# pierremtb/PINNs-TF2.0

Hardware: AMD Instinct MI355X
Metric: collocation-points/sec (higher is better)
Workload: dtype f64

## Files before the change

include/pinn_hip.h:

```cpp
#ifndef PINN_HIP_H
#define PINN_HIP_H

#include <stdint.h>

#ifdef __cplusplus
extern "C" {
#endif

typedef struct pinn_ctx pinn_ctx;

enum {
  PINN_PDE_BURGERS = 0,
  PINN_PDE_BURGERS_IDE = 1,
  PINN_PDE_SCHRODINGER = 2,
  PINN_PDE_BURGERS_DISC = 3,
  PINN_PDE_BURGERS_DISC_IDE = 4,
  PINN_PDE_ADR = 5,
  PINN_PDE_ADR_IDE = 6
};
enum { PINN_F32 = 0, PINN_F64 = 1 };
enum {
  PINN_OK = 0, PINN_EINVAL = -1, PINN_EHIP = -2, PINN_ESTATE = -3, PINN_ECOMM = -4,
  PINN_EUNSUPPORTED = -5
};

const char* pinn_last_error(void);
int pinn_abi_version(void);
int pinn_device_count(int* n);
int pinn_runtime_versions(int* hip_runtime, int* hip_driver, int* rccl);
int pinn_device_info(int device, char* name, int cap, int* n_cu, int64_t* hbm_bytes);

int pinn_create(pinn_ctx** out, const int* layers, int n_layers, const double* lb,
                const double* ub, int pde_kind, int dtype, int device);
int pinn_destroy(pinn_ctx* c);
int pinn_num_params(pinn_ctx* c, int64_t* n);

int pinn_set_collocation(pinn_ctx* c, const double* X_f, int64_t n, int64_t n_total);
int pinn_set_data(pinn_ctx* c, const double* X_u, const double* u, int64_t n, int64_t n_total);
int pinn_lhs_collocation(pinn_ctx* c, int64_t n_design, int64_t first, int64_t count, uint64_t seed);
int pinn_get_collocation(pinn_ctx* c, double* X, int64_t n);
int pinn_rad_collocation(pinn_ctx* c, int64_t n_design, int64_t first, int64_t count, int64_t n_pool, uint64_t seed,
                         int k, double c_add);
int pinn_set_boundary(pinn_ctx* c, const double* X_lb, const double* X_ub, int64_t n,
                      int64_t n_total);
int pinn_disc_set_stage(pinn_ctx* c, int set, const double* x, const double* target, int64_t n,
                        const double* M, int q);
int pinn_disc_predict(pinn_ctx* c, int set, const double* x, int64_t n, double* out);

int pinn_set_pde_params(pinn_ctx* c, const double* p, int n);
int pinn_get_pde_params(pinn_ctx* c, double* p, int n);
int pinn_set_pde_trainable(pinn_ctx* c, int mask);

int pinn_set_weights(pinn_ctx* c, const double* w, int64_t n);
int pinn_get_weights(pinn_ctx* c, double* w, int64_t n);

int pinn_loss_grad(pinn_ctx* c, double* loss, double* grad, double* terms);

int pinn_adam_init(pinn_ctx* c, double lr, double beta1, double beta2, double eps);
int pinn_adam_run(pinn_ctx* c, int n_steps, double* losses);
int pinn_adam_run_terms(pinn_ctx* c, int n_steps, double* terms3);

int pinn_lbfgs_begin(pinn_ctx* c, int max_iter, double lr, int n_corr, double tol_fun,
                     double tol_x, double max_eval);
int pinn_lbfgs_run(pinn_ctx* c, int n_iters, int* iters, double* losses, int* n_logged,
                   int* done);
int pinn_adam_enqueue(pinn_ctx* c, int n_steps, int* ticket);
int pinn_adam_enqueue_terms(pinn_ctx* c, int n_steps, int* ticket);
int pinn_adam_collect(pinn_ctx* c, int ticket, double* losses);
int pinn_lbfgs_enqueue(pinn_ctx* c, int n_iters, int* ticket);
int pinn_lbfgs_collect(pinn_ctx* c, int ticket, int cap, int* iters, double* losses, int* n_logged, int* done);
int pinn_weights_snapshot(pinn_ctx* c, int slot);
int pinn_weights_restore(pinn_ctx* c, int slot);
int pinn_lbfgs_set_mode(pinn_ctx* c, int mode);
int pinn_lbfgs_get_x(pinn_ctx* c, double* x, int64_t n);

int pinn_predict(pinn_ctx* c, const double* X, int64_t n, double* out);
int pinn_error_l2(pinn_ctx* c, const double* X, const double* ref, int64_t n, int kind, double* err);
int pinn_residual(pinn_ctx* c, double* f, int64_t n);
int pinn_residual_at(pinn_ctx* c, const double* X, int64_t n, double* f);

int pinn_get_status(pinn_ctx* c, int64_t* n_evals, int64_t* first_nonfinite_eval);

int pinn_comm_unique_id(char* id128);
int pinn_comm_init(pinn_ctx* c, const char* id128, int n_ranks, int rank);
int pinn_comm_xgmi_export(pinn_ctx* c, int n_ranks, int rank, char* handle64);
int pinn_comm_xgmi_attach(pinn_ctx* c, const char* handles, int n_handles, int* mapped_ok);
int pinn_comm_xgmi_selftest(pinn_ctx* c, int* ok);
int pinn_comm_benchmark(pinn_ctx* c, int mode, int iters, double* us_per_iter);
int pinn_comm_set_mode(pinn_ctx* c, int mode);
int pinn_comm_get_mode(pinn_ctx* c, int* mode);

int pinn_timing_enable(pinn_ctx* c, int max_evals, int every);
int pinn_timing_read(pinn_ctx* c, double* avg_ms, int* n);
int pinn_sync(pinn_ctx* c);
int pinn_set_kernel_path(pinn_ctx* c, int path);
int pinn_get_kernel_path(pinn_ctx* c, int* path);
int pinn_debug_stamps(pinn_ctx* c, long long* out, int64_t cap, int64_t* n_waves);
int pinn_debug_coef_stamps(long long* out16);
int pinn_debug_t16f_stamps(long long* out512);
int pinn_debug_t16_deal(int W, int* out49);

typedef struct pinn_ens pinn_ens;
int pinn_ens_create(pinn_ens** out, const int* layers, int n_layers, const double* lb, const double* ub, int pde_kind,
                    int dtype, int device, int n_members);
int pinn_ens_destroy(pinn_ens* e);
int pinn_ens_size(pinn_ens* e, int* n_members, int64_t* n_params);
int pinn_ens_set_collocation(pinn_ens* e, const double* X_f, int64_t n, int64_t n_total);
int pinn_ens_set_data(pinn_ens* e, const double* X_u, const double* u, int64_t n, int64_t n_total);
int pinn_ens_set_pde_params(pinn_ens* e, const double* p, int n);
int pinn_ens_set_weights(pinn_ens* e, const double* w, int64_t n);
int pinn_ens_get_weights(pinn_ens* e, double* w, int64_t n);
int pinn_ens_loss_grad(pinn_ens* e, double* losses, double* grads, double* terms);
int pinn_ens_adam_init(pinn_ens* e, double lr, double beta1, double beta2, double eps, const double* lr_k);
int pinn_ens_adam_run(pinn_ens* e, int n_steps, double* losses);
int pinn_ens_lbfgs_begin(pinn_ens* e, int n_corr, double tol_fun, double tol_x, double max_eval, double lr,
                         const double* lr_k, int max_iter, const int* max_iter_k);
int pinn_ens_lbfgs_run(pinn_ens* e, int n_iters, int* iters, double* losses, int* n_logged, int* done);
int pinn_ens_predict(pinn_ens* e, const double* X, int64_t n, double* out);
int pinn_ens_error_l2(pinn_ens* e, const double* X, const double* ref, int64_t n, double* err);
int pinn_ens_get_status(pinn_ens* e, int64_t* n_evals, int64_t* first_nonfinite_eval);

int pinn_ensk_set_collocation(pinn_ens* e, const double* X_f, int64_t n, int64_t n_total);
int pinn_ensk_set_data(pinn_ens* e, const double* X_u, const double* u, int64_t n, int64_t n_total);
int pinn_ensk_set_pde_params(pinn_ens* e, const double* nu, int n_members);
int pinn_ensk_lhs_collocation(pinn_ens* e, int64_t n_design, int64_t first, int64_t count, const uint64_t* seeds);

int pinn_sa_set_weights(pinn_ctx* c, const double* lam_u, int64_t n_u, const double* lam_f, int64_t n_f);
int pinn_sa_get_weights(pinn_ctx* c, double* lam_u, int64_t n_u, double* lam_f, int64_t n_f);
int pinn_sa_adam_init(pinn_ctx* c, double lr);
int pinn_sa_disable(pinn_ctx* c);

int pinn_pw_set(pinn_ctx* c, const double* lam_u, int64_t n_u, const double* lam_f, int64_t n_f, const double* lam_b,
                int64_t n_b);
int pinn_pw_get(pinn_ctx* c, double* lam_u, int64_t n_u, double* lam_f, int64_t n_f, double* lam_b, int64_t n_b);
int pinn_pw_adam_init(pinn_ctx* c, double rate_u, double rate_f, double rate_b);
int pinn_pw_disable(pinn_ctx* c);

int pinn_set_robin(pinn_ctx* c, const double* X_w , const double* alpha, const double* beta, const double* g,
                   int64_t n, int64_t n_total);
int pinn_robin_residual(pinn_ctx* c, double* out , int64_t n);

int pinn_set_source(pinn_ctx* c, const double* s , int64_t n);

int pinn_set_coef_fields(pinn_ctx* c, const double* K , int64_t n);

#ifdef __cplusplus
}
#endif
#endif
```

pinns-tf2.0_amd/csrc/engine.hip:

```cpp
#include <hip/hip_runtime.h>
#include <rccl/rccl.h>

#include <cmath>
#include <cstdarg>
#include <cstddef>
#include <cstdio>
#include <cstring>
#include <string>
#include <chrono>
#include <vector>

#include "../../include/pinn_hip.h"
#include "kernels_fused20.h"
#include "kernels_fused20m.h"
#include "fused20d_api.h"
#include "fused20m_api.h"
#include "kernels_wide.h"
#include "kernels_generic.h"
#include "kernels_optim.h"
#include "kernels_disc.h"
#include "kernels_sampling.h"
#include "kernels_rad.h"
#include "kernels_tile16.h"
#include "kernels_tile16f.h"
// ... 26 lines not shown

#define NCCLCHK(expr)                                                                     \
  do {                                                                                    \
    ncclResult_t r_ = (expr);                                                             \
    if (r_ != ncclSuccess)                                                                \
      return fail(PINN_ECOMM, "%s failed: %s (%s:%d)", #expr, ncclGetErrorString(r_),     \
                  __FILE__, __LINE__);                                                    \
  } while (0)

#define REQUIRE(cond, ...)                                \
  do {                                                    \
    if (!(cond)) return fail(PINN_EINVAL, __VA_ARGS__);   \
  } while (0)

struct Roctx {
  int (*push)(const char*) = nullptr;
  int (*pop)() = nullptr;
  Roctx() {
    if (getenv("PINN_NO_ROCTX")) return;
    void* h = dlopen("librocprofiler-sdk-roctx.so", RTLD_LAZY | RTLD_GLOBAL);
    if (!h) h = dlopen("librocprofiler-sdk-roctx.so.1", RTLD_LAZY | RTLD_GLOBAL);
    if (!h) return;
    push = (int (*)(const char*))dlsym(h, "roctxRangePushA");
    pop = (int (*)())dlsym(h, "roctxRangePop");
    if (!push || !pop) push = nullptr, pop = nullptr;
  }
};
static Roctx& roctx() { static Roctx r; return r; }
struct Range {
  bool on;
  explicit Range(const char* name) : on(roctx().push != nullptr) { if (on) roctx().push(name); }
  ~Range() { if (on) roctx().pop(); }
};

static constexpr int CHUNK_POINTS = 32768;
static constexpr int LOSS_SLOTS = 4;

enum KernelPath : int {
  KP_GENERIC = 0,
  KP_FUSED20 = 1,
  KP_FUSED20M = 2,
  KP_WIDE = 3,
  KP_T16 = 4,
  KP_T16_FWD = 5,
  KP_T16_BWD = 6,
  KP_FUSED20D = 7,
  KP_T16_FUSED = 8,
  KP_COUNT
};

enum { LAM_PAIRS, LAM_DATA, LAM_COL, LAM_CLASSES };
struct LamStore {
  double* buf = nullptr;
  size_t cap = 0;
  int n_hdr = 0;
  double hdr[PW_CONST] = {0.0, 0.0, 0.0, 0.0, 0.0, 0.0, 0.0, 0.0};
  int n[LAM_CLASSES] = {0, 0, 0};
  bool reset[LAM_CLASSES] = {false, false, false};
};

struct pinn_ctx {
  int device = 0, dtype = PINN_F32, pde = PINN_PDE_BURGERS;
  KernelPath path = KP_GENERIC;
  hipStream_t stream = nullptr;
  bool own_stream = true;
  NetDesc nd{};
  int layers[MAX_DENSE + 1]{};
  int n_layers = 0;
  double lb[2]{}, ub[2]{}, nu = 0.0;
  double adr[6]{};
  int adr_mask = 0;

  std::vector<double> Xf, Xu, U, Xlo, Xhi;
  int64_t nf_total = 0, nu_total = 0, nb_total = 0;
  bool sets_dirty = true;
  SetDesc sd{};

  void *xs = nullptr, *ts = nullptr, *tgt = nullptr;
  double *theta = nullptr, *gl = nullptr, *adam_m = nullptr, *adam_v = nullptr;
  void* theta_r = nullptr;
  float* img = nullptr;
  int* row_index = nullptr;
  int n_cu = 256, n_wg = 0;
  void *S = nullptr, *O = nullptr, *ZA = nullptr, *ZB = nullptr, *part = nullptr;
  size_t cap_S = 0, cap_O = 0, cap_Z = 0, cap_part = 0, cap_pts = 0;
  int chunk = 0, n_rows = 0, R = 0;
  void *xe = nullptr, *te = nullptr, *Oe = nullptr;
  size_t cap_eval = 0;
  double* f_out = nullptr;
  size_t cap_f = 0;
  std::vector<double> ev_X, ev_ref;
  int ev_n_pad = 0;
  double *pred = nullptr, *d_ref = nullptr, *err_partial = nullptr, *err_res = nullptr;
  size_t cap_pred = 0, cap_ref = 0, cap_errp = 0;
  double* h_err = nullptr;
  unsigned long long* d_nonfinite = nullptr;
  unsigned long long n_evals = 0;

  double lr = 1e-3, b1 = 0.9, b2 = 0.999, eps = 1e-7;
  int64_t adam_t = 0;
  bool adam_ready = false, adam_want_terms = false;
  double* loss_hist = nullptr;
  size_t cap_loss_hist = 0;

  struct Pending {
    int kind = 0;
    int n = 0;
    int base = 0, issued_upto = 0;
    bool want_terms = false;
    hipEvent_t ev = nullptr;
    double* h_loss = nullptr; size_t cap_loss = 0;
    int* h_iter = nullptr; size_t cap_iter = 0;
    LbfgsState* h_state = nullptr;
  };
  static constexpr int N_SNAP = 4;
  double* snap = nullptr;
  unsigned snap_valid = 0;
  static constexpr int N_PENDING = 4;
  Pending pend[N_PENDING];
  unsigned long long tickets_issued = 0, tickets_collected = 0;
  int lb_issued_at_read = 0;

  LbfgsState* lb_state = nullptr;
  int lb_flip = 0;
  double *lb_x = nullptr, *lb_d = nullptr, *lb_gold = nullptr, *lb_S = nullptr, *lb_Y = nullptr,
         *lb_ro = nullptr, *lb_al = nullptr, *lb_q = nullptr, *lb_log_loss = nullptr;
  int* lb_log_iter = nullptr;
  int lb_max_iter = 0, lb_ncorr = 0, lb_cap_corr = 0, lb_cap_log = 0, lb_logged_read = 0;
  double lb_lr = 1.0, lb_tol_fun = 0, lb_tol_x = 0, lb_max_eval = 0;
  int lb_iters_issued = 0;
  bool lb_post_pending = false;
  bool lb_ready = false;
  int lb_mode = 1, lb_mode_active = 0, lb_M1 = 0;
  double *lb_SY = nullptr, *lb_YY = nullptr, *lb_dots = nullptr, *lb_cs = nullptr, *lb_cy = nullptr;
  LbcExtra* lb_ex = nullptr;
  double t16_cost_full = T16_COST_FULL, t16_cost_strip = T16_COST_STRIP;
  long long t16_handover_ticks = 50000000ll;
  bool t16_prepass_pinned = false;
  bool t16_prepass = false;
  unsigned int* t16_bsync = nullptr;
  unsigned int t16_bcount = 0;
  double* t16_gscr = nullptr;
  size_t t16_gscr_bytes = 0;

  struct { bool on = false; int64_t n_design = 0, first = 0, count = 0; uint64_t seed = 0; } lhs;
  struct {
    bool on = false, filled = false;
    int64_t n_design = 0, first = 0, count = 0;
    double *cx = nullptr, *ct = nullptr;
    size_t cap = 0;
    void *px = nullptr, *pt = nullptr, *O = nullptr;
    double* f = nullptr;
    unsigned long long *w = nullptr, *bsum = nullptr;
    RadTotals* tot = nullptr;
    size_t cap_pool = 0;
  } rad;

  struct {
    bool on = false;
    double lr = 0.0;
    LamStore arr;
  } sa;
  struct {
    bool on = false;
    double rate[3] = {0.0, 0.0, 0.0};
    LamStore arr;
// ... 471 lines not shown
                               (int)lds));
  hipLaunchKernelGGL((k_t16_fwd<real, NT, WLDS, NWV>), dim3(t16_wgs(c, pts)), dim3(64 * NWV), lds, c->stream, c->nd,
                     (const real*)c->theta_r, (const real*)xs, (const real*)ts, base, n_pad, chunk,
                     pts / 16, lbx, lbt, sx, st, (vec4<real>*)c->S, (vec4<real>*)O);
  return 0;
}
template <typename real, int NT, int PDE, bool WLDS>
static int t16_launch_bwd(pinn_ctx* c, int base, int pts, real lbx, real lbt, real sx, real st, int accumulate) {
  static unsigned long long attr = 0;
  constexpr int NWV = (NT == 8 && !WLDS) ? 8 : 4;
  const size_t lds = t16_bwd_lds<NT>(sizeof(real), WLDS);
  if (first_call_on_device(attr))
    HIPCHK(hipFuncSetAttribute((const void*)k_t16_bwd<real, NT, PDE, WLDS, NWV>, hipFuncAttributeMaxDynamicSharedMemorySize,
                               (int)lds));
  const int rows_cap = t16_wgs(c, c->chunk);
  const int wgs = t16_wgs(c, pts) < rows_cap ? t16_wgs(c, pts) : rows_cap;
  hipLaunchKernelGGL((k_t16_bwd<real, NT, PDE, WLDS, NWV>), dim3(wgs), dim3(64 * NWV), lds, c->stream, c->nd, c->sd,
                     (const real*)c->theta_r, (const real*)c->xs, (const real*)c->ts, (const real*)c->tgt, base,
                     c->sd.n_pad, c->chunk, pts / 16, lbx, lbt, sx, st, (real)c->nu, (const vec4<real>*)c->S,
                     (const vec4<real>*)c->O, (real*)c->part, c->R, accumulate);
  return 0;
}
template <typename real>
static int t16_fwd(pinn_ctx* c, const void* xs, const void* ts, int n_pad, int chunk, void* O, int base, int pts,
                   real lbx, real lbt, real sx, real st) {
  if (c->nd.width > 64)
    return t16_launch_fwd<real, 8, false>(c, xs, ts, n_pad, chunk, O, base, pts, lbx, lbt, sx, st);
  if (!t16_lds_weights(c, pts))
    return t16_launch_fwd<real, 4, false>(c, xs, ts, n_pad, chunk, O, base, pts, lbx, lbt, sx, st);
  return t16_launch_fwd<real, 4, true>(c, xs, ts, n_pad, chunk, O, base, pts, lbx, lbt, sx, st);
}
template <typename real>
static int forward_chunk(pinn_ctx* c, const void* xs, const void* ts, int n_pad, int chunk, void* O, int base, int pts) {
  const real lbx = (real)c->lb[0], lbt = (real)c->lb[1];
  const real sx = (real)(2.0 / (c->ub[0] - c->lb[0])), st = (real)(2.0 / (c->ub[1] - c->lb[1]));
  if (tile16_ok(c) && c->nd.width >= 24)
    return t16_fwd<real>(c, xs, ts, n_pad, chunk, O, base, pts, lbx, lbt, sx, st);
  constexpr int JT = sizeof(real) == 4 ? 20 : 10;
  hipLaunchKernelGGL((k_forward<real, JT>), dim3(pts / 64), dim3(64), 0, c->stream, c->nd, (const real*)c->theta_r,
                     (const real*)xs, (const real*)ts, base, n_pad, chunk, lbx, lbt, sx, st, (vec4<real>*)c->S,
                     (vec4<real>*)O);
  return 0;
}

template <typename real, int PDE>
static int t16_bwd(pinn_ctx* c, int base, int pts, real lbx, real lbt, real sx, real st, int accumulate) {
  if (c->nd.width > 64)
    return t16_launch_bwd<real, 8, PDE, false>(c, base, pts, lbx, lbt, sx, st, accumulate);
  if (!t16_lds_weights(c, pts))
    return t16_launch_bwd<real, 4, PDE, false>(c, base, pts, lbx, lbt, sx, st, accumulate);
  return t16_launch_bwd<real, 4, PDE, true>(c, base, pts, lbx, lbt, sx, st, accumulate);
}

template <int PDE, int H>
static int t16_fused_launch(pinn_ctx* c, const SetDesc& sd, int base, int pts, int ci, int wgs, int n_bg, double lbx,
                            double lbt, double sx, double st) {
  static unsigned long long attr = 0;
  if (first_call_on_device(attr))
    HIPCHK(hipFuncSetAttribute((const void*)k_t16_fused<PDE, H>, hipFuncAttributeMaxDynamicSharedMemorySize,
                               160 * 1024));
  hipLaunchKernelGGL((k_t16_fused<PDE, H>), dim3(wgs), dim3(512), t16_fused_lds(c->nd.width, H, c->nd.n_out), c->stream, c->nd, sd,
                     (const double*)c->theta_r, (const double*)c->xs, (const double*)c->ts, (const double*)c->tgt, base,
                     sd.n_pad, pts / 16, lbx, lbt, sx, st, (double)c->nu, (vec4<double>*)c->O, (double*)c->part, c->R,
                     ci > 0 ? 1 : 0, c->t16_bsync, c->t16_bcount, n_bg, c->t16_gscr, c->t16_handover_ticks,
                     t16_deal(c->nd.width, c->t16_cost_full, c->t16_cost_strip));
  HIPCHK(hipGetLastError());
  return 0;
}

template <typename real>
struct InMap {
  real lbx, lbt, sx, st;
  explicit InMap(const pinn_ctx* c)
      : lbx((real)c->lb[0]), lbt((real)c->lb[1]), sx((real)(2.0 / (c->ub[0] - c->lb[0]))), st((real)(2.0 / (c->ub[1] - c->lb[1]))) {}
};

static F20dLaunch fused20d_args(const pinn_ctx* c, hipEvent_t* ev4) {
  const InMap<double> m(c);
  return F20dLaunch{c->nd, c->sd, (const double*)c->theta_r, (const double*)c->xs, (const double*)c->ts,
                    (const double*)c->tgt, m.lbx, m.lbt, m.sx, m.st, (double*)c->part, c->R, c->n_wg, 1, c->row_index,
                    c->stream, c->stamps, ev4 ? ev4[0] : nullptr, ev4 ? ev4[1] : nullptr};
}

template <typename real, int PDE>
static int launch_fused20d(pinn_ctx* c, hipEvent_t* ev4, const AdamFuse* af) {
  int rc = hipErrorInvalidValue;
  if constexpr (sizeof(real) == 8 && PDE != 2) {
    const bool weighted = PDE == 0 && c->sa.on;
    if (weighted) { if (int e = lam_prepare(c, c->sa.arr, sa_layout(c))) return e; }
    const bool pw = PDE == PDE_ADR && c->pw.on;
    if (pw) { if (int e = lam_prepare(c, c->pw.arr, pw_layout(c))) return e; }
    const F20dLaunch a = fused20d_args(c, ev4);
    if constexpr (PDE == PDE_ADR) {
      if (pw) rc = fused20d_launch_any(a, AdrPwArgs{pde_coef<double, PDE_ADR>(c), c->pw.arr.buf, af ? af->bc_pw : 0.0});
      else rc = fused20d_launch_any(a, pde_coef<double, PDE_ADR>(c));
    }
    else if constexpr (PDE == PDE_ADR_ROBIN) rc = fused20d_launch_any(a, pde_coef<double, PDE_ADR_ROBIN>(c));
    else if constexpr (PDE == PDE_ADR_SRC) rc = fused20d_launch_any(a, pde_coef<double, PDE_ADR_SRC>(c));
    else if constexpr (PDE == PDE_ADR_VAR) rc = fused20d_launch_any(a, pde_coef<double, PDE_ADR_VAR>(c));
    else if constexpr (PDE == PDE_ADR_IDE) rc = fused20d_launch_any(a, pde_coef<double, PDE_ADR_IDE>(c));
    else if (weighted) rc = fused20d_launch_any(a, SaArgs{(double)c->nu, c->sa.arr.buf, af ? af->alpha_sa : 0.0});
    else rc = fused20d_launch_any(PDE, a, (double)c->nu);
  }
  if (rc) return fail(PINN_EHIP, "fused20d launch failed: %s", hipGetErrorString((hipError_t)rc));
  return 0;
}

template <typename real, int PDE>
static int launch_fused20m(pinn_ctx* c, hipEvent_t* ev4) {
  int rc = hipErrorInvalidValue;
  if constexpr (sizeof(real) == 4 && PDE != 2 && !pde_is_adr(PDE)) {
    const InMap<float> m(c);
    hipEvent_t const e0 = ev4 ? ev4[0] : nullptr, e1 = ev4 ? ev4[1] : nullptr;
    if (c->nd.n_hidden == 8)
      rc = fused20m_launch<PDE, 8>(c->nd, c->sd, (const float*)c->theta_r, c->img, (const float*)c->xs,
                                   (const float*)c->ts, (const float*)c->tgt, m.lbx, m.lbt, m.sx, m.st, (float)c->nu,
                                   (float*)c->part, c->R, c->n_wg, c->stream, c->stamps, e0, e1);
    else
      rc = fused20m_launch_depth(PDE, c->nd, c->sd, (const float*)c->theta_r, c->img, (const float*)c->xs,
                                 (const float*)c->ts, (const float*)c->tgt, m.lbx, m.lbt, m.sx, m.st, (float)c->nu,
                                 (float*)c->part, c->R, c->n_wg, c->stream, c->stamps, e0, e1);
  }
  if (rc) return fail(PINN_EHIP, "fused20m launch failed: %s", hipGetErrorString((hipError_t)rc));
  return 0;
}

template <typename real, int PDE>
static int launch_fused20(pinn_ctx* c, hipEvent_t* ev4) {
  int rc = hipErrorInvalidValue;
  if constexpr (!pde_is_adr(PDE)) {
    const InMap<real> m(c);
    rc = fused20_launch<real, PDE>(c->nd, c->sd, (const real*)c->theta_r, (const real*)c->xs, (const real*)c->ts,
                                   (const real*)c->tgt, m.lbx, m.lbt, m.sx, m.st, (real)c->nu, (vec4<real>*)c->S,
                                   (real*)c->part, c->R, c->stream, c->stamps, ev4 ? ev4[0] : nullptr,
                                   ev4 ? ev4[1] : nullptr);
  }
  if (rc) return fail(PINN_EHIP, "fused20 launch failed: %s", hipGetErrorString((hipError_t)rc));
  return 0;
}

template <typename real, int PDE>
static int chunk_t16_fused(pinn_ctx* c, const InMap<real>& m, hipEvent_t ev1, int base, int pts, int ci) {
  if constexpr (sizeof(real) == 8 && !pde_is_adr(PDE)) {
    const SetDesc& sd = c->sd;
    const int rows_cap = t16_wgs(c, c->chunk);
    const int wgs = t16_wgs(c, pts) < rows_cap ? t16_wgs(c, pts) : rows_cap;
    int n_bg = (PDE == 2 && base == 0 && sd.n_b > 0) ? (2 * sd.n_b + 15) / 16 : 0;
    REQUIRE(wgs >= 1 && wgs <= pts / 16 && (ci > 0 || wgs == rows_cap),
            "k_t16_fused launch plan: %d workgroups for %d groups (rows %d, chunk %d)", wgs, pts / 16, rows_cap, ci);
    if (n_bg > wgs || (n_bg > 0 && c->t16_prepass)) {
      const size_t need_S = (size_t)c->nd.n_hidden * c->nd.width * (size_t)c->chunk * 4 * sizeof(double);
      if (need_S > c->cap_S) { if (dev_alloc(&c->S, need_S)) return PINN_EHIP; c->cap_S = need_S; }
      if (int rc = t16_fwd<real>(c, c->xs, c->ts, sd.n_pad, c->chunk, c->O, 0, 16 * n_bg < pts ? 16 * n_bg : pts, m.lbx, m.lbt, m.sx, m.st)) return rc;
      n_bg = 0;
    }
    if (!c->t16_bsync) {
      if (dev_alloc(&c->t16_bsync, 64)) return PINN_EHIP;
      HIPCHK(hipMemsetAsync(c->t16_bsync, 0, 64, c->stream));
      c->t16_bcount = 0;
    }
    c->t16_bcount += (unsigned int)n_bg;
    {
      const size_t ntl = ((size_t)c->nd.width + 15) / 16;
      const size_t need = (size_t)rows_cap * (c->nd.n_hidden - 1) * ntl * ntl * 256 * sizeof(double);
      if (need > c->t16_gscr_bytes) {
        if (dev_alloc(&c->t16_gscr, need)) return PINN_EHIP;
        c->t16_gscr_bytes = need;
      }
    }
    if (ev1) HIPCHK(hipEventRecord(ev1, c->stream));
    switch (c->nd.n_hidden) {
      case 2: return t16_fused_launch<PDE, 2>(c, sd, base, pts, ci, wgs, n_bg, m.lbx, m.lbt, m.sx, m.st);
      case 3: return t16_fused_launch<PDE, 3>(c, sd, base, pts, ci, wgs, n_bg, m.lbx, m.lbt, m.sx, m.st);
      case 4: return t16_fused_launch<PDE, 4>(c, sd, base, pts, ci, wgs, n_bg, m.lbx, m.lbt, m.sx, m.st);
    }
// ... 525 lines not shown
int pinn_abi_version(void) { return 6; }

int pinn_device_count(int* n) {
  REQUIRE(n, "null");
  HIPCHK(hipGetDeviceCount(n));
  return 0;
}

int pinn_runtime_versions(int* hip_runtime, int* hip_driver, int* rccl) {
  if (hip_runtime) HIPCHK(hipRuntimeGetVersion(hip_runtime));
  if (hip_driver) HIPCHK(hipDriverGetVersion(hip_driver));
  if (rccl) {
    const ncclResult_t r = ncclGetVersion(rccl);
    if (r != ncclSuccess) return fail(PINN_ECOMM, "ncclGetVersion: %s", ncclGetErrorString(r));
  }
  return 0;
}

int pinn_device_info(int device, char* name, int cap, int* n_cu, int64_t* hbm_bytes) {
  hipDeviceProp_t p;
  HIPCHK(hipGetDeviceProperties(&p, device));
  if (name && cap > 0) snprintf(name, cap, "%s (%s)", p.name, p.gcnArchName);
  if (n_cu) *n_cu = p.multiProcessorCount;
  if (hbm_bytes) *hbm_bytes = (int64_t)p.totalGlobalMem;
  return 0;
}

static int adr_ide_write_tail(pinn_ctx* c, const double* p) {
  double tail[6];
  for (int i = 0; i < 6; ++i) tail[i] = i == 2 ? std::log(p[i]) : p[i];
  HIPCHK(hipSetDevice(c->device));
  HIPCHK(hipMemcpyAsync(c->theta + c->nd.n_net, tail, sizeof(tail), hipMemcpyHostToDevice, c->stream));
  HIPCHK(hipStreamSynchronize(c->stream));
  if (int rc = cast_weights(c)) return rc;
  HIPCHK(hipStreamSynchronize(c->stream));
  return 0;
}

int pinn_create(pinn_ctx** out, const int* layers, int n_layers, const double* lb,
                const double* ub, int pde_kind, int dtype, int device) {
  REQUIRE(out && layers && lb && ub, "null argument");
  REQUIRE(n_layers >= 3 && n_layers <= MAX_DENSE + 1, "need 3..%d layer sizes, got %d", MAX_DENSE + 1, n_layers);
  REQUIRE(dtype == PINN_F32 || dtype == PINN_F64, "dtype must be PINN_F32 or PINN_F64");
  REQUIRE(pde_kind >= 0 && pde_kind <= PINN_PDE_ADR_IDE, "unknown pde kind %d", pde_kind);
  const bool disc = pde_kind == PINN_PDE_BURGERS_DISC || pde_kind == PINN_PDE_BURGERS_DISC_IDE;
  if (disc) REQUIRE(layers[0] == 1, "discrete-time models take one input (x), got %d", layers[0]);
  else REQUIRE(layers[0] == 2, "input dimension must be 2 (x, t), got %d", layers[0]);
  const int W = layers[1], NO = layers[n_layers - 1];
  for (int i = 1; i < n_layers - 1; ++i)
    REQUIRE(layers[i] == W, "all hidden widths must be equal (the reference's sizes_w assumes it, "
                            "utils/neuralnetwork.py:40-45); got %d vs %d", layers[i], W);
  REQUIRE(W >= 1 && W <= MAX_WIDTH, "hidden width %d outside 1..%d", W, MAX_WIDTH);
  if (disc) {
    REQUIRE(NO >= 1 && NO <= 65536, "output size %d outside 1..65536", NO);
    REQUIRE(W <= (dtype == PINN_F64 ? 64 : 128), "discrete-time models: hidden width %d exceeds what the LDS-resident "
            "kernels hold (64 in float64, 128 in float32)", W);
  }
  else REQUIRE(NO == (pde_kind == PINN_PDE_SCHRODINGER ? 2 : 1), "output size %d does not match the PDE kind", NO);
  REQUIRE(ub[0] > lb[0] && (disc || ub[1] > lb[1]), "ub must exceed lb");
  int ndev = 0;
  HIPCHK(hipGetDeviceCount(&ndev));
  REQUIRE(device >= 0 && device < ndev, "device %d not present (%d devices)", device, ndev);
  HIPCHK(hipSetDevice(device));

  pinn_ctx* c = new pinn_ctx();
  c->device = device; c->dtype = dtype; c->pde = pde_kind; c->n_layers = n_layers;
  for (int i = 0; i < n_layers; ++i) c->layers[i] = layers[i];
  c->lb[0] = lb[0]; c->ub[0] = ub[0];
  if (disc) { c->lb[1] = 0.0; c->ub[1] = 1.0; } else { c->lb[1] = lb[1]; c->ub[1] = ub[1]; }
  c->nu = 0.01 / M_PI;
  c->adr[1] = 1.0; c->adr[2] = c->nu;
  NetDesc& nd = c->nd;
  nd.n_hidden = n_layers - 2; nd.width = W; nd.n_out = NO;
  int off = 0;
  for (int d = 0; d < n_layers - 1; ++d) {
    nd.off_w[d] = off; off += layers[d] * layers[d + 1];
    nd.off_b[d] = off; off += layers[d + 1];
  }
  nd.n_net = off;
  nd.n_theta = off + tail_len(pde_kind);
  c->R = nd.n_theta + LOSS_SLOTS;
  hipError_t e = hipStreamCreateWithFlags(&c->stream, hipStreamNonBlocking);
  if (e != hipSuccess) { delete c; return fail(PINN_EHIP, "hipStreamCreate: %s", hipGetErrorString(e)); }
  if (const char* v = getenv("PINN_T16_PREPASS")) {
    if (!(v[0] == '0' || v[0] == '1') || v[1]) { delete c; return fail(PINN_EINVAL, "PINN_T16_PREPASS must be 0 or 1 (got \"%s\")", v); }
    c->t16_prepass = v[0] == '1';
    c->t16_prepass_pinned = true;
  }
  if (const char* v = getenv("PINN_T16_HANDOVER_TICKS")) {
    char* end = nullptr;
    const long long t = strtoll(v, &end, 10);
    if (end == v || *end || t <= 0) { delete c; return fail(PINN_EINVAL, "PINN_T16_HANDOVER_TICKS must be a positive integer of 100 MHz ticks (got \"%s\")", v); }
    c->t16_handover_ticks = t;
  }
  if (const char* v = getenv("PINN_T16_COSTS")) {
    double a = 0, b = 0;
    char tail = 0;
    if (sscanf(v, "%lf,%lf%c", &a, &b, &tail) != 2 || !(a > 0 && b > 0)) { delete c; return fail(PINN_EINVAL, "PINN_T16_COSTS must be two positive numbers \"full,strip\" (got \"%s\")", v); }
    c->t16_cost_full = a; c->t16_cost_strip = b;
  }
  const size_t n = nd.n_theta;
  if (dev_alloc(&c->theta, n * 8) || dev_alloc(&c->gl, (size_t)c->R * 8) ||
      dev_alloc(&c->adam_m, n * 8) || dev_alloc(&c->adam_v, n * 8) ||
      dev_alloc(&c->theta_r, n * real_size(c) + 1024)) { delete c; return PINN_EHIP; }
  HIPCHK(hipMemsetAsync(c->theta, 0, n * 8, c->stream));
  HIPCHK(hipMemsetAsync(c->theta_r, 0, n * real_size(c), c->stream));
  HIPCHK(hipMemsetAsync(c->gl, 0, (size_t)c->R * 8, c->stream));
  if (dev_alloc(&c->d_nonfinite, 8)) { delete c; return PINN_EHIP; }
  HIPCHK(hipMemsetAsync(c->d_nonfinite, 0, 8, c->stream));
  HIPCHK(hipStreamSynchronize(c->stream));
  {
    hipDeviceProp_t prop;
    if (hipGetDeviceProperties(&prop, device) == hipSuccess && prop.multiProcessorCount > 0)
      c->n_cu = prop.multiProcessorCount;
  }
  if (fused_regs_ok(c)) {
    const size_t nimg = fused20m_image_floats(nd.n_hidden);
    if (dev_alloc(&c->img, nimg * 4)) { delete c; return PINN_EHIP; }
    HIPCHK(hipMemsetAsync(c->img, 0, nimg * 4, c->stream));
    HIPCHK(hipStreamSynchronize(c->stream));
  }
  if (fused_regs_ok(c)) nd.img_kind = 1;
  if (fused_f64_ok(c)) {
    std::vector<int> ri((size_t)fused20d_blocks(nd.n_hidden) * 16);
    fused20d_row_index(nd, nd.n_hidden, ri.data());
    if (dev_alloc(&c->row_index, ri.size() * sizeof(int))) { delete c; return PINN_EHIP; }
    HIPCHK(hipMemcpy(c->row_index, ri.data(), ri.size() * sizeof(int), hipMemcpyHostToDevice));
  }
  if (wide_ok(c)) {
    const size_t nimg = wide_image_floats<100>(nd.n_hidden);
    if (dev_alloc(&c->img, nimg * 4)) { delete c; return PINN_EHIP; }
    HIPCHK(hipMemsetAsync(c->img, 0, nimg * 4, c->stream));
    HIPCHK(hipStreamSynchronize(c->stream));
    nd.img_kind = 2;
  }
  for (KernelPath p : PATH_PREFERENCE)
    if (path_ok(c, p)) { c->path = p; break; }
  if (is_adr_ide(c)) {
    if (int rc = adr_ide_write_tail(c, c->adr)) { pinn_destroy(c); return rc; }
  }
  *out = c;
  return 0;
}

int pinn_destroy(pinn_ctx* c) {
  if (!c) return 0;
  (void)hipSetDevice(c->device);
  (void)hipStreamSynchronize(c->stream);
  if (c->comm) ncclCommDestroy(c->comm);
  xg_release(c);
  void* ptrs[] = {c->xs, c->ts, c->tgt, c->theta, c->gl, c->adam_m, c->adam_v, c->theta_r, c->S,
                  c->O, c->ZA, c->ZB, c->part, c->xe, c->te, c->Oe, c->f_out, c->loss_hist, c->snap,
                  c->lb_state, c->lb_x, c->lb_d, c->lb_gold, c->lb_S, c->lb_Y, c->lb_ro, c->lb_al,
                  c->lb_q, c->lb_log_loss, c->lb_log_iter, c->lb_SY, c->lb_YY, c->lb_dots, c->lb_cs,
                  c->lb_cy, c->lb_ex, c->img, c->row_index, c->sa.arr.buf, c->pw.arr.buf, c->d_ginfo, c->d_M[0], c->d_M[1], c->d_MT[0], c->d_MT[1],
                  c->d_Ast, c->d_A3, c->d_U3, c->d_Nn, c->d_R, c->d_dAp, c->d_lossp, c->d_lamp,
                  c->pred, c->d_ref, c->err_partial, c->err_res, c->d_nonfinite, c->t16_bsync, c->t16_gscr,
                  c->rad.cx, c->rad.ct, c->rad.px, c->rad.pt, c->rad.O, c->rad.f, c->rad.w, c->rad.bsum, c->rad.tot,
                  c->robin.ab, c->robin.out, c->kf.dev};
  for (void* p : ptrs) if (p) (void)hipFree(p);
  for (auto& p : c->pend) {
    if (p.h_state) (void)hipHostFree(p.h_state);
    if (p.h_loss) (void)hipHostFree(p.h_loss);
    if (p.h_iter) (void)hipHostFree(p.h_iter);
    if (p.ev) (void)hipEventDestroy(p.ev);
  }
// ... 1054 lines not shown
  return 0;
}

int pinn_timing_enable(pinn_ctx* c, int max_evals, int every) {
  REQUIRE(c && max_evals >= 0 && every >= 1, "bad arguments");
  HIPCHK(hipSetDevice(c->device));
  while ((int)c->ev.size() < 4 * (max_evals > 8 ? max_evals : 8)) {
    hipEvent_t e;
    HIPCHK(hipEventCreate(&e));
    c->ev.push_back(e);
  }
  if (max_evals > 0) {
    HIPCHK(hipStreamSynchronize(c->stream));
    for (int i = 0; i < 16; ++i) HIPCHK(hipEventRecord(c->ev[i], c->stream));
    HIPCHK(hipStreamSynchronize(c->stream));
    double acc = 0;
    for (int i = 2; i < 16; i += 2) {
      float ms = 0;
      HIPCHK(hipEventElapsedTime(&ms, c->ev[i], c->ev[i + 1]));
      acc += ms;
    }
    c->ev_overhead_ms = acc / 7.0;
  }
  c->ev_cap_evals = max_evals; c->ev_used = 0; c->timing = max_evals > 0;
  c->ev_every = every; c->ev_seen = 0;
  return 0;
}

int pinn_timing_read(pinn_ctx* c, double* avg_ms, int* n) {
  REQUIRE(c && avg_ms && n, "null");
  HIPCHK(hipSetDevice(c->device));
  HIPCHK(hipStreamSynchronize(c->stream));
  double a = 0, b = 0, t = 0;
  for (int i = 0; i < c->ev_used; ++i) {
    float m01 = 0, m02 = 0, m03 = 0;
    HIPCHK(hipEventElapsedTime(&m01, c->ev[4 * i], c->ev[4 * i + 1]));
    HIPCHK(hipEventElapsedTime(&m02, c->ev[4 * i], c->ev[4 * i + 2]));
    HIPCHK(hipEventElapsedTime(&m03, c->ev[4 * i], c->ev[4 * i + 3]));
    a += m01; b += m02; t += m03;
  }
  *n = c->ev_used;
  const double k = c->ev_used ? 1.0 / c->ev_used : 0.0;
  avg_ms[0] = a * k; avg_ms[1] = b * k; avg_ms[2] = t * k; avg_ms[3] = c->ev_overhead_ms;
  avg_ms[4] = PATHS[c->path].one_launch ? 1.0 : 0.0;
  c->ev_used = 0;
  return 0;
}

int pinn_sync(pinn_ctx* c) {
  REQUIRE(c, "null");
  HIPCHK(hipSetDevice(c->device));
  HIPCHK(hipStreamSynchronize(c->stream));
  return xg_check(c);
}

int pinn_set_kernel_path(pinn_ctx* c, int path) {
  REQUIRE(c && (unsigned)path < (unsigned)KP_COUNT, "path must be 0 (generic), 1 (fused width-20), 2 (fused width-20, register stash), "
          "3 (wide MFMA sweeps), 4 (shape-generic MFMA sweeps), 5 / 6 (4's forward / reverse half with the generic other half), "
          "7 (fused width-20 float64, register stash), 8 (fused float64 MFMA sweep, widths 65..128, 2-4 hidden layers)");
  const KernelPath p = (KernelPath)path;
  if (c->sa.on && p != KP_FUSED20D)
    return fail(PINN_EUNSUPPORTED, "pinn_set_kernel_path: self-adaptive weights run on kernel path 7 only (pinn_sa_disable first)");
  if (c->pw.on && p != KP_FUSED20D)
    return fail(PINN_EUNSUPPORTED, "pinn_set_kernel_path: point weights run on kernel path 7 only (pinn_pw_disable first)");
  if (is_adr(c) && !adr_has_path(p))
    return fail(PINN_EUNSUPPORTED, "pinn_set_kernel_path: the adr kind (pde 5) runs on kernel paths 0 and 7 only; path %d "
                "(%s) has no variant for it", path, PATHS[p].name);
  if (is_adr_ide(c) && !adr_has_path(p))
    return fail(PINN_EUNSUPPORTED, "pinn_set_kernel_path: the adr_ide kind (pde 6) runs on kernel paths 0 and 7 only; path %d "
                "(%s) has no variant for it", path, PATHS[p].name);
  REQUIRE(PATHS[p].ok(c), "%s", PATHS[p].needs);
  c->path = p;
  c->sets_dirty = true;
  return 0;
}

int pinn_debug_stamps(pinn_ctx* c, long long* out, int64_t cap, int64_t* n_waves) {
#ifdef PINN_STAMPS
  REQUIRE(c && out && n_waves, "null");
  REQUIRE(c->path != KP_GENERIC, "stamps exist for the fused kernels only");
  HIPCHK(hipSetDevice(c->device));
  int rc = ensure_sets(c);
  if (rc) return rc;
  const size_t n = (size_t)path_rows(c) * 4 * 32;
  REQUIRE((size_t)cap >= n, "stamp buffer too small: need %zu", n);
  if (dev_alloc(&c->stamps, n * 8)) return PINN_EHIP;
  HIPCHK(hipMemsetAsync(c->stamps, 0, n * 8, c->stream));
  rc = eval_loss_grad(c);
  if (rc) return rc;
  HIPCHK(hipMemcpyAsync(out, c->stamps, n * 8, hipMemcpyDeviceToHost, c->stream));
  HIPCHK(hipStreamSynchronize(c->stream));
  (void)hipFree(c->stamps);
  c->stamps = nullptr;
  *n_waves = (int64_t)(n / 32);
  return 0;
#else
  (void)c; (void)out; (void)cap; (void)n_waves;
  return fail(PINN_EUNSUPPORTED, "built without -DPINN_STAMPS (profiling build only)");
#endif
}

int pinn_debug_coef_stamps(long long* out16) {
#ifdef PINN_STAMPS
  REQUIRE(out16, "null");
  HIPCHK(hipDeviceSynchronize());
  HIPCHK(hipMemcpyFromSymbol(out16, HIP_SYMBOL(g_coef_stamps), 16 * sizeof(long long)));
  return 0;
#else
  (void)out16;
  return fail(PINN_EUNSUPPORTED, "built without -DPINN_STAMPS (profiling build only)");
#endif
}

int pinn_debug_t16_deal(int W, int* out49) {
  REQUIRE(out49 && W >= 1 && W <= 128, "width outside 1..128");
  const T16Deal d = t16_deal(W);
  for (int w = 0; w < 8; ++w) {
    out49[w] = d.f_lo[w]; out49[8 + w] = d.f_hi[w]; out49[16 + w] = d.e_lo[w]; out49[24 + w] = d.e_hi[w];
    out49[32 + w] = d.row0[w]; out49[40 + w] = d.ns[w];
  }
  out49[48] = d.edge;
  return 0;
}

int pinn_debug_t16f_stamps(long long* out512) {
#ifdef PINN_STAMPS
  REQUIRE(out512, "null");
  HIPCHK(hipDeviceSynchronize());
  HIPCHK(hipMemcpyFromSymbol(out512, HIP_SYMBOL(g_t16f_stamps), 8 * 64 * sizeof(long long)));
  return 0;
#else
  (void)out512;
  return fail(PINN_EUNSUPPORTED, "built without -DPINN_STAMPS (profiling build only)");
#endif
}

int pinn_get_kernel_path(pinn_ctx* c, int* path) {
  REQUIRE(c && path, "null");
  *path = c->path;
  return 0;
}

static int sa_supported(const pinn_ctx* c, const char* who) {
  if (c->pde != PINN_PDE_BURGERS)
    return fail(PINN_EUNSUPPORTED, "%s: self-adaptive weights are for Burgers inference (pde 0) only", who);
  if (c->dtype != PINN_F64) return fail(PINN_EUNSUPPORTED, "%s: self-adaptive weights need float64", who);
  if (c->path != KP_FUSED20D)
    return fail(PINN_EUNSUPPORTED, "%s: self-adaptive weights need kernel path 7 (this context runs path %d)", who, (int)c->path);
  if (c->comm || c->xg.box)
    return fail(PINN_EUNSUPPORTED, "%s: self-adaptive weights are single-device; this context has a communicator", who);
  return 0;
}

static void sa_counts(const pinn_ctx* c, int64_t* n_u, int64_t* n_f) {
  *n_u = (int64_t)(c->Xu.size() / 2);
  *n_f = c->lhs.on ? c->lhs.count : c->rad.on ? c->rad.count : (int64_t)(c->Xf.size() / 2);
}

int pinn_sa_set_weights(pinn_ctx* c, const double* lam_u, int64_t n_u, const double* lam_f, int64_t n_f) {
  REQUIRE(c, "null");
  if (int rc = sa_supported(c, "pinn_sa_set_weights")) return rc;
  int64_t cu, cf;
  sa_counts(c, &cu, &cf);
  REQUIRE((lam_u || n_u == 0) && (lam_f || n_f == 0), "pinn_sa_set_weights: null weight array");
  REQUIRE(n_u == cu && n_f == cf, "pinn_sa_set_weights: %lld / %lld weights for %lld data and %lld collocation points",
          (long long)n_u, (long long)n_f, (long long)cu, (long long)cf);
  for (int64_t j = 0; j < n_u; ++j) REQUIRE(std::isfinite(lam_u[j]), "pinn_sa_set_weights: lam_u[%lld] is not finite", (long long)j);
  for (int64_t i = 0; i < n_f; ++i) REQUIRE(std::isfinite(lam_f[i]), "pinn_sa_set_weights: lam_f[%lld] is not finite", (long long)i);
  HIPCHK(hipSetDevice(c->device));
  if (int rc = ensure_sets(c)) return rc;
  const LamLayout L = sa_layout(c);
  std::vector<double> h(L.doubles(), 0.0);
  for (int64_t j = 0; j < n_u; ++j) h[L.at(LAM_DATA) + 3 * j] = lam_u[j];
  for (int64_t i = 0; i < n_f; ++i) h[L.at(LAM_COL) + 3 * i] = lam_f[i];
  if (int rc = lam_upload(c, c->sa.arr, L, h)) return rc;
  c->sa.on = true;
  return 0;
}

int pinn_sa_get_weights(pinn_ctx* c, double* lam_u, int64_t n_u, double* lam_f, int64_t n_f) {
  REQUIRE(c, "null");
  REQUIRE(c->sa.on, "pinn_sa_get_weights: self-adaptive weights are off (pinn_sa_set_weights)");
  int64_t cu, cf;
  sa_counts(c, &cu, &cf);
  REQUIRE((lam_u || n_u == 0) && (lam_f || n_f == 0), "pinn_sa_get_weights: null weight array");
  REQUIRE(n_u == cu && n_f == cf, "pinn_sa_get_weights: %lld / %lld weights for %lld data and %lld collocation points",
          (long long)n_u, (long long)n_f, (long long)cu, (long long)cf);
  HIPCHK(hipSetDevice(c->device));
  if (int rc = ensure_sets(c)) return rc;
  const LamLayout L = sa_layout(c);
  if (int rc = lam_prepare(c, c->sa.arr, L)) return rc;
  std::vector<double> h;
  if (int rc = lam_download(c, c->sa.arr, h)) return rc;
  for (int64_t j = 0; j < n_u; ++j) lam_u[j] = h[L.at(LAM_DATA) + 3 * j];
  for (int64_t i = 0; i < n_f; ++i) lam_f[i] = h[L.at(LAM_COL) + 3 * i];
  return 0;
}

int pinn_sa_adam_init(pinn_ctx* c, double lr) {
  REQUIRE(c, "null");
  if (int rc = sa_supported(c, "pinn_sa_adam_init")) return rc;
  REQUIRE(std::isfinite(lr) && lr >= 0.0, "pinn_sa_adam_init: lr %g must be finite and >= 0", lr);
  c->sa.lr = lr;
  return 0;
}

int pinn_sa_disable(pinn_ctx* c) {
  REQUIRE(c, "null");
  c->sa.on = false;
  return 0;
}

static int pw_supported(const pinn_ctx* c, const char* who) {
  if (c->pde != PINN_PDE_ADR) return fail(PINN_EUNSUPPORTED, "%s: point weights are for the adr kind (pde 5) only", who);
  if (c->dtype != PINN_F64) return fail(PINN_EUNSUPPORTED, "%s: point weights need float64", who);
  if (c->path != KP_FUSED20D)
    return fail(PINN_EUNSUPPORTED, "%s: point weights need kernel path 7 (this context runs path %d)", who, (int)c->path);
  if (c->comm || c->xg.box)
    return fail(PINN_EUNSUPPORTED, "%s: point weights are single-device; this context has a communicator", who);
  return 0;
}

// ... 518 lines not shown
```

pinns-tf2.0_amd/csrc/fused20d_api.h:

```cpp
#pragma once
#include <hip/hip_runtime.h>
#include "kernels_generic.h"

namespace pinn {

constexpr int fused20d_blocks(int H) { return 5 + (H - 1) * 30 + 6; }
inline size_t fused20d_weight_doubles(int n_theta) { return ((size_t)n_theta + 127) / 128 * 128; }
#ifndef PINN_ONETILE_SUM
#define PINN_ONETILE_SUM 0
#endif
constexpr int FUSED20D_STAGE_WAVE = PINN_ONETILE_SUM ? 30 * 16 : 30 * 64;
constexpr int FUSED20D_STAGE_BUF = 4 * FUSED20D_STAGE_WAVE;
constexpr int fused20d_stage_doubles(int n_hidden) {
  return PINN_ONETILE_SUM == 2 ? fused20d_blocks(n_hidden) * 64 : 2 * FUSED20D_STAGE_BUF;
}
inline size_t fused20d_lds_bytes(int n_hidden, int n_theta) {
  const size_t acc = (size_t)4 * fused20d_blocks(n_hidden) * 16, stage = (size_t)fused20d_stage_doubles(n_hidden);
  return (fused20d_weight_doubles(n_theta) + (acc > stage ? acc : stage) + 4 * 256) * sizeof(double);
}

void fused20d_row_index(const NetDesc& nd, int H, int* out);

inline bool fused20d_depth_ok(int n_hidden) { return n_hidden == 4 || n_hidden == 6 || n_hidden == 8; }

struct F20dLaunch {
  const NetDesc& nd;
  const SetDesc& sd;
  const double* th;
  const double *xs, *ts, *tgt;
  double lbx, lbt, sx, st;
  double* part;
  int R, n_wg, n_members;
  const int* row_index;
  hipStream_t stream;
  long long* stamps;
  hipEvent_t ev_start, ev_stop;
};

int fused20d_launch_any(int pde, const F20dLaunch& a, double nu);

int fused20d_ens_launch_any(int pde, const F20dLaunch& a, double nu);

int fused20d_ens_launch_any(int pde, const F20dLaunch& a, const double* nu_k);

constexpr int SA_CONST = 4;
struct SaArgs {
  double nu;
  double* lam;
  double alpha;
};

int fused20d_launch_any(const F20dLaunch& a, const SaArgs& sa);

int fused20d_launch_any(const F20dLaunch& a, const AdrCoef<double>& k);

int fused20d_launch_any(const F20dLaunch& a, const AdrIdeArg& k);

constexpr int PW_CONST = 8;
struct AdrPwArgs {
  AdrCoef<double> k;
  double* lam;
  double bc;
};
int fused20d_launch_any(const F20dLaunch& a, const AdrPwArgs& k);

int fused20d_launch_any(const F20dLaunch& a, const AdrRobinArg<double>& k);

int fused20d_launch_any(const F20dLaunch& a, const AdrSrcArg<double>& k);

int fused20d_launch_any(const F20dLaunch& a, const AdrVarArg<double>& k);

}
```

pinns-tf2.0_amd/csrc/kernels_fused20d.h:

```cpp
#pragma once
#include <hip/hip_ext.h>
#include <type_traits>
#include "kernels_fused20.h"
#include "fused20d_api.h"

#ifndef PINN_FOLD_STAGES
#define PINN_FOLD_STAGES 1
#endif
#ifndef PINN_GACC_ATOMIC
#define PINN_GACC_ATOMIC 1
#endif
static_assert(PINN_FOLD_STAGES == 1 || PINN_FOLD_STAGES == 2, "PINN_FOLD_STAGES: 1 (product) or 2; the unfolded form is retired");
#ifndef PINN_ROW_STORE_WT
#define PINN_ROW_STORE_WT 1
#endif

#if defined(PINN_STAMPS) && defined(PINN_STAMPS2)
#define STAMP2(cond, i) do { if (cond) STAMP(i); } while (0)
#else
#define STAMP2(cond, i) do { } while (0)
#endif

namespace pinn {


struct agd { int lo, hi; };
__device__ __forceinline__ agd agd_put(const double x) {
  agd a;
  const int lo = __double2loint(x), hi = __double2hiint(x);
  asm("v_accvgpr_write_b32 %0, %1" : "=a"(a.lo) : "v"(lo));
  asm("v_accvgpr_write_b32 %0, %1" : "=a"(a.hi) : "v"(hi));
  return a;
}
__device__ __forceinline__ agd agd_put_after(const double x, const double after) {
  agd a;
  const int lo = __double2loint(x), hi = __double2hiint(x), dep = __double2hiint(after);
  asm("v_accvgpr_write_b32 %0, %1" : "=a"(a.lo) : "v"(lo), "v"(dep));
  asm("v_accvgpr_write_b32 %0, %1" : "=a"(a.hi) : "v"(hi), "v"(dep));
  return a;
}
__device__ __forceinline__ double agd_get(const agd a) {
  int lo, hi;
  asm("v_accvgpr_read_b32 %0, %1" : "=v"(lo) : "a"(a.lo));
  asm("v_accvgpr_read_b32 %0, %1" : "=v"(hi) : "a"(a.hi));
  return __hiloint2double(hi, lo);
}

__device__ __forceinline__ double mfma444(const double a, const double b, const double c) {
  return __builtin_amdgcn_mfma_f64_4x4x4f64(a, b, c, 0, 0, 0);
}

constexpr int DPP_ROW_ROR4 = 0x124, DPP_ROW_ROR8 = 0x128;

__device__ __forceinline__ double bit_pick(const int m, const double a, const double b) {
  const int lo = (__double2loint(a) & m) | (__double2loint(b) & ~m), hi = (__double2hiint(a) & m) | (__double2hiint(b) & ~m);
  return __hiloint2double(hi, lo);
}


__device__ __forceinline__ double tanh_d(const double x) {
  const double t = exp(-2.0 * fabs(x));
  const double y = 1.0 + t;
  double r = __builtin_amdgcn_rcp(y);
  r = __builtin_fma(__builtin_fma(-y, r, 1.0), r, r);
  r = __builtin_fma(__builtin_fma(-y, r, 1.0), r, r);
  const double num = 1.0 - t;
  double qv = num * r;
  qv = __builtin_fma(__builtin_fma(-y, qv, num), r, qv);
  return copysign(qv, x);
}

__device__ __forceinline__ void channels_d(const double a, const double zp, const double zq, const double zr,
                                           double& h, double& p, double& q, double& r) {
  const double d1 = __builtin_fma(-a, a, 1.0);
  const double t = (-2.0 * a) * zp;
  h = a; p = d1 * zp; q = d1 * zq; r = d1 * __builtin_fma(t, zp, zr);
}

__device__ __forceinline__ void preact_adjoint_d(const double a, const double zp, const double zq, const double zr,
                                                 const double oh, const double op, const double oq, const double orr,
                                                 double& bh, double& bp, double& bq, double& br) {
  const double a2 = a * a, d1 = 1.0 - a2;
  const double d2 = (-2.0 * a) * d1;
  const double d3 = (-2.0 * d1) * __builtin_fma(-3.0, a2, 1.0);
  const double zpw = zp * orr;
  const double dot = __builtin_fma(zr, orr, __builtin_fma(zq, oq, zp * op));
  bh = __builtin_fma(d3 * zp, zpw, __builtin_fma(d2, dot, d1 * oh));
  bp = __builtin_fma(d2 + d2, zpw, d1 * op);
  bq = d1 * oq;
  br = d1 * orr;
}

template <bool SETS, bool SAW = false, int PDE = 0>
using f20d_nu_t = typename std::conditional<PDE == PDE_ADR_VAR, AdrVarArg<double>, typename std::conditional<PDE == PDE_ADR_SRC, AdrSrcArg<double>, typename std::conditional<PDE == PDE_ADR_ROBIN, AdrRobinArg<double>, typename std::conditional<PDE == PDE_ADR && SAW, AdrPwArgs, typename std::conditional<PDE == PDE_ADR, AdrCoef<double>, typename std::conditional<PDE == PDE_ADR_IDE, AdrIdeArg, typename std::conditional<SETS, const double*, typename std::conditional<SAW, SaArgs, double>::type>::type>::type>::type>::type>::type>::type>::type;
__device__ __forceinline__ double f20d_nu(double nu) { return nu; }
__device__ __forceinline__ double f20d_nu(const AdrIdeArg&) { return 0.0; }
__device__ __forceinline__ double f20d_nu(const AdrCoef<double>& k) { return k.nu; }
__device__ __forceinline__ double f20d_nu(const double* nu) { return nu[blockIdx.y]; }
__device__ __forceinline__ double f20d_nu(const SaArgs& a) { return a.nu; }
__device__ __forceinline__ double f20d_nu(const AdrPwArgs& a) { return a.k.nu; }
__device__ __forceinline__ double f20d_nu(const AdrRobinArg<double>& a) { return a.k.nu; }

#define PINN_F20D_KERNEL k_fused20d
#include "kernels_fused20d_kernel.h"
#undef PINN_F20D_KERNEL
#define PINN_F20D_KERNEL k_robin20d
#include "kernels_fused20d_kernel.h"
#undef PINN_F20D_KERNEL
#define PINN_F20D_KERNEL k_src20d
#include "kernels_fused20d_kernel.h"
#undef PINN_F20D_KERNEL
#define PINN_F20D_KERNEL k_var20d
#include "kernels_fused20d_kernel.h"
#undef PINN_F20D_KERNEL
template <int PDE, int H, bool ONE_TILE, bool ENS, bool SETS, bool SAW>
constexpr auto f20d_kernel() {
  if constexpr (PDE == PDE_ADR_ROBIN) return &k_robin20d<PDE, H, ONE_TILE, ENS, SETS, SAW>;
  else if constexpr (PDE == PDE_ADR_SRC) return &k_src20d<PDE, H, ONE_TILE, ENS, SETS, SAW>;
  else if constexpr (PDE == PDE_ADR_VAR) return &k_var20d<PDE, H, ONE_TILE, ENS, SETS, SAW>;
  else return &k_fused20d<PDE, H, ONE_TILE, ENS, SETS, SAW>;
}

template <int PDE, int H, bool ENS, bool SETS, bool SAW>
inline int fused20d_launch(const F20dLaunch& a, const f20d_nu_t<SETS, SAW, PDE>& nu) {
  if (!w20_layout_ok(a.nd, H, pde_n_tail(PDE)) || (!ENS && a.n_members != 1)) return (int)hipErrorInvalidValue;
  const size_t lds = fused20d_lds_bytes(H, a.nd.n_theta);
  static unsigned long long attr_set = 0;
  if (first_call_on_device(attr_set)) {
    hipError_t e = hipFuncSetAttribute((const void*)f20d_kernel<PDE, H, false, ENS, SETS, SAW>(),
                                       hipFuncAttributeMaxDynamicSharedMemorySize, (int)lds);
    if (e == hipSuccess)
      e = hipFuncSetAttribute((const void*)f20d_kernel<PDE, H, true, ENS, SETS, SAW>(),
                              hipFuncAttributeMaxDynamicSharedMemorySize, (int)lds);
    if (e != hipSuccess) return (int)e;
  }
  const int n_tiles = a.sd.n_pad / 64;
  auto* const kern = a.n_wg >= n_tiles ? f20d_kernel<PDE, H, true, ENS, SETS, SAW>() : f20d_kernel<PDE, H, false, ENS, SETS, SAW>();
  const dim3 grid(a.n_wg, a.n_members);
  if (a.ev_start && a.ev_stop)
    hipExtLaunchKernelGGL(kern, grid, dim3(256), lds, a.stream, a.ev_start, a.ev_stop, 0, a.th, a.xs, a.ts, a.tgt, a.part,
                          a.row_index, a.R, n_tiles, a.lbx, a.lbt, a.sx, a.st, nu, a.sd, a.stamps, w20_desc(H, pde_n_tail(PDE)));
  else
    hipLaunchKernelGGL(kern, grid, dim3(256), lds, a.stream, a.th, a.xs, a.ts, a.tgt, a.part, a.row_index, a.R, n_tiles,
                       a.lbx, a.lbt, a.sx, a.st, nu, a.sd, a.stamps, w20_desc(H, pde_n_tail(PDE)));
  return (int)hipGetLastError();
}

}
```

pinns-tf2.0_amd/csrc/kernels_fused20d_kernel.h:

```cpp
template <int PDE, int H, bool ONE_TILE, bool ENS = false, bool SETS = false, bool SAW = false>
__global__ __launch_bounds__(256) void PINN_F20D_KERNEL(const double* __restrict__ th, const double* __restrict__ xs,
                                                  const double* __restrict__ ts, const double* __restrict__ tgt,
                                                  double* __restrict__ part, const int* __restrict__ row_index, int R,
                                                  int n_tiles, double lbx, double lbt, double sx, double st,
                                                  f20d_nu_t<SETS, SAW, PDE> nu, SetDesc sd,
                                                  long long* __restrict__ stamps, W20Desc nd_arg) {
  static_assert(ENS || !SETS, "per-member point sets are an ensemble launch");
  static_assert(!pde_is_adr(PDE) || (!ENS && !SETS && (!SAW || PDE == PDE_ADR)),
                "advection-diffusion-reaction: solo launch; point weights for the fixed-coefficient kind only");
  static_assert(!SAW || ((PDE == 0 || PDE == PDE_ADR) && !ENS), "point weights: Burgers inference or adr, solo launch");
  static_assert(PDE != PDE_ADR_ROBIN || (!ENS && !SETS && !SAW),
                "Robin points: the fixed-coefficient adr kind only, solo launch, no point weights");
  static_assert(PDE != PDE_ADR_SRC || (!ENS && !SETS && !SAW),
                "source term: the fixed-coefficient adr kind only, solo launch, no point weights");
  static_assert(PDE != PDE_ADR_VAR || (!ENS && !SETS && !SAW),
                "coefficient fields: the adr kind only, solo launch, no point weights (no SAW)");
  constexpr W20Desc nd_const = w20_desc(H, pde_n_tail(PDE));
  const W20Desc nd = ONE_TILE ? nd_const : nd_arg;
  constexpr int NBLK = fused20d_blocks(H);
  constexpr int BLK_H = 5 + (H - 1) * 30;
  extern __shared__ __attribute__((aligned(16))) unsigned char lds_raw[];
  double* const wl = reinterpret_cast<double*>(lds_raw);
  const int nwp = (nd.n_theta + 127) / 128 * 128;
  if constexpr (ENS) {
    th += (size_t)blockIdx.y * nwp;
    part += (size_t)blockIdx.y * gridDim.x * R;
    if constexpr (SETS) {
      const size_t po = (size_t)blockIdx.y * sd.n_pad;
      xs += po; ts += po; tgt += po;
    }
  }
  double* const gacc_all = wl + nwp;
  double* const lacc_all = gacc_all + (ONE_TILE ? fused20d_stage_doubles(H) : 4 * NBLK * 16);

#define PINN_TO_POINTS(X) mfma444((X), ident, 0.0)
  STAMP(0);
  const int tid = threadIdx.x;
  const int wave = __builtin_amdgcn_readfirstlane(tid >> 6);
#define PINN_LANE_INDICES(L)                                                                                          \
  const int lane = (L);                                                                                                \
  const int q = lane & 15;                                                               \
  const int s = lane >> 4;                                                 \
  const int i4 = lane & 3;                        \
  const int pf = s * FW + i4;                                               \
  const int pr = i4 * FW + s;                                               \
  const double ident = s == i4 ? 1.0 : 0.0;                     \
  const int ge = s * 4 + i4;                                        \
  double* const lacc = lacc_all + wave * 256 + lane;                             \
  const int sput = (s * 4 + i4) * 4 + ((lane >> 2) & 3);    \
  const double onesA = i4 == 0 ? 1.0 : 0.0;                      \
  (void)q; (void)pf; (void)pr; (void)ident; (void)ge; (void)lacc; (void)onesA; (void)s; (void)sput
  PINN_LANE_INDICES(tid & 63);
  double* const gacc = gacc_all + wave * (NBLK * 16);

  int tile = blockIdx.x;
  double x = 0.0, t = 0.0;
  if (tile < n_tiles) { x = xs[tile * 64 + wave * 16 + q]; t = ts[tile * 64 + wave * 16 + q]; }

  for (int c = wave; c < nwp / 128; c += 4)
    __builtin_amdgcn_global_load_lds((const __attribute__((address_space(1))) void*)(th + c * 128 + lane * 2),
                                     (__attribute__((address_space(3))) void*)(wl + c * 128), 16, 0, 0);
  {
    typedef double d2 __attribute__((ext_vector_type(2)));
    if (ONE_TILE) {
      d2* const z = reinterpret_cast<d2*>(lacc_all);
      for (int i = tid; i < 2 * 256; i += 256) z[i] = d2{0.0, 0.0};
    } else {
      d2* const z = reinterpret_cast<d2*>(gacc_all);
      for (int i = tid; i < 2 * NBLK * 16 + 2 * 256; i += 256) z[i] = d2{0.0, 0.0};
    }
  }
  asm volatile("s_waitcnt vmcnt(0)" ::: "memory");
  __syncthreads();

  double c1 = 1.0, c2 = f20d_nu(nu);
  if (PDE == 1) { c1 = wl[nd.n_net]; c2 = exp(wl[nd.n_net + 1]); }
  double* sa_lam_p = nullptr;
  double sa_alpha = 0.0;
  if constexpr (SAW) {
    sa_lam_p = nu.lam;
    if constexpr (PDE == PDE_ADR) sa_alpha = nu.bc; else sa_alpha = nu.alpha;
    if constexpr (!ONE_TILE) asm volatile("" : "+v"(sa_lam_p), "+v"(sa_alpha));
  }
  const double inv_nf = sd.inv_nf, inv_nu = sd.inv_nu;
  double* adr_park = nullptr;
  if constexpr (PDE == PDE_ADR && !ONE_TILE && !SAW) {
    adr_park = lacc_all + wave * 256 + 192;
    if ((tid & 63) == 0) {
      adr_park[0] = nu.a0; adr_park[1] = nu.a1; adr_park[2] = nu.nu; adr_park[3] = nu.r1; adr_park[4] = nu.r2;
      adr_park[5] = nu.r3; adr_park[6] = sd.inv_nb;
    }
  }
  const double* rb_ab = nullptr;
  if constexpr (pde_adr_robin(PDE)) {
    rb_ab = nu.ab;
    if constexpr (!ONE_TILE) {
      asm volatile("" : "+v"(rb_ab));
      adr_park = lacc_all + wave * 256 + 192;
      if ((tid & 63) == 0) {
        adr_park[0] = nu.k.a0; adr_park[1] = nu.k.a1; adr_park[2] = nu.k.nu; adr_park[3] = nu.k.r1; adr_park[4] = nu.k.r2;
        adr_park[5] = nu.k.r3; adr_park[6] = sd.inv_nb; adr_park[7] = (double)nu.first; adr_park[8] = (double)nu.n;
        adr_park[9] = nu.inv_nw;
      }
    }
  }
  (void)rb_ab;
  const double* kf_tab = nullptr;
  if constexpr (PDE == PDE_ADR_VAR) {
    kf_tab = nu.kf;
    if constexpr (!ONE_TILE) asm volatile("" : "+v"(kf_tab));
  }
  (void)kf_tab;
  if constexpr (PDE == PDE_ADR_IDE) {
    adr_park = lacc_all + wave * 256 + 192;
    if ((tid & 63) == 0) {
      const double* const tail = wl + nd.n_theta - 6;
      adr_park[0] = tail[0]; adr_park[1] = tail[1]; adr_park[2] = exp(tail[2]); adr_park[3] = tail[3]; adr_park[4] = tail[4];
      adr_park[5] = tail[5]; adr_park[6] = sd.inv_nb; adr_park[7] = (double)nu.mask;
    }
  }
  if constexpr (PDE == PDE_ADR && SAW) {
    adr_park = lacc_all + wave * 256 + 192;
    const AdrCoef<double> k0 = nu.k;
    if ((tid & 63) == 0) {
      adr_park[0] = k0.a0; adr_park[1] = k0.a1; adr_park[2] = k0.nu; adr_park[3] = k0.r1; adr_park[4] = k0.r2;
      adr_park[5] = k0.r3; adr_park[6] = sd.inv_nb;
    }
    if ((tid & 63) < PW_CONST) adr_park[8 + (tid & 63)] = sa_lam_p[tid & 63];
  }
  (void)adr_park;


  STAMP(1);

  for (; tile < n_tiles; tile += gridDim.x) {
    PINN_LANE_INDICES(tid & 63);
    auto grad_fetch = [&](const int blk) { return (ONE_TILE || PINN_GACC_ATOMIC) ? 0.0 : gacc[blk * 16 + ge]; };
    int phase_first = 0;
    constexpr int PARK_BLOCK = 1;
    constexpr int STAGE_WAVE_STRIDE = PINN_ONETILE_SUM ? 1 : FUSED20D_STAGE_WAVE;
#if PINN_ONETILE_SUM == 2
#define PINN_PHASE_STAGE(P) ((P) == 0 ? BLK_H : (P) == H ? 0 : 5 + (H - (P) - 1) * 30) * 64
#else
#define PINN_PHASE_STAGE(P) ((P) & 1) * FUSED20D_STAGE_BUF
#endif
    double* stage_w = gacc_all + wave * STAGE_WAVE_STRIDE;
    constexpr unsigned long long FOLD_LANES = PINN_FOLD_STAGES == 2 ? 0x000f000f000f000full : 0x00ff00ff00ff00ffull;
    double pend_D[6] = {0, 0, 0, 0, 0, 0};
    int pend_off[6] = {0, 0, 0, 0, 0, 0}, pend_n = 0;
    auto gacc_flush = [&]() {
#if PINN_GACC_ATOMIC
      if constexpr (!ONE_TILE) {
        const unsigned addr = (unsigned)(uintptr_t)(__attribute__((address_space(3))) void*)(gacc + ge);
        unsigned long long saved;
        if (pend_n == 6)
          asm volatile("s_mov_b64 %[sv], exec\n\ts_mov_b64 exec, %[mk]\n\t"
                       "ds_add_f64 %[a], %[d0] offset:%[o0]\n\tds_add_f64 %[a], %[d1] offset:%[o1]\n\t"
                       "ds_add_f64 %[a], %[d2] offset:%[o2]\n\tds_add_f64 %[a], %[d3] offset:%[o3]\n\t"
                       "ds_add_f64 %[a], %[d4] offset:%[o4]\n\tds_add_f64 %[a], %[d5] offset:%[o5]\n\t"
                       "s_mov_b64 exec, %[sv]"
                       : [sv] "=&s"(saved)
                       : [a] "v"(addr), [mk] "s"(FOLD_LANES), [d0] "v"(pend_D[0]), [d1] "v"(pend_D[1]),
                         [d2] "v"(pend_D[2]), [d3] "v"(pend_D[3]), [d4] "v"(pend_D[4]), [d5] "v"(pend_D[5]),
                         [o0] "i"(pend_off[0]), [o1] "i"(pend_off[1]), [o2] "i"(pend_off[2]), [o3] "i"(pend_off[3]),
                         [o4] "i"(pend_off[4]), [o5] "i"(pend_off[5])
                       : "memory");
        else
          asm volatile("s_mov_b64 %[sv], exec\n\ts_mov_b64 exec, %[mk]\n\t"
                       "ds_add_f64 %[a], %[d0] offset:%[o0]\n\tds_add_f64 %[a], %[d1] offset:%[o1]\n\t"
                       "ds_add_f64 %[a], %[d2] offset:%[o2]\n\tds_add_f64 %[a], %[d3] offset:%[o3]\n\t"
                       "ds_add_f64 %[a], %[d4] offset:%[o4]\n\t"
                       "s_mov_b64 exec, %[sv]"
                       : [sv] "=&s"(saved)
                       : [a] "v"(addr), [mk] "s"(FOLD_LANES), [d0] "v"(pend_D[0]), [d1] "v"(pend_D[1]),
                         [d2] "v"(pend_D[2]), [d3] "v"(pend_D[3]), [d4] "v"(pend_D[4]),
                         [o0] "i"(pend_off[0]), [o1] "i"(pend_off[1]), [o2] "i"(pend_off[2]), [o3] "i"(pend_off[3]),
                         [o4] "i"(pend_off[4])
                       : "memory");
      }
#endif
#if PINN_ONETILE_SUM
      if constexpr (ONE_TILE) {
        const unsigned addr = (unsigned)(uintptr_t)(__attribute__((address_space(3))) void*)(stage_w + ge * 4);
        constexpr unsigned long long park = 0x000f000f000f000full << (4 * PARK_BLOCK);
        unsigned long long saved;
        if (pend_n == 6)
          asm volatile("s_mov_b64 %[sv], exec\n\ts_mov_b64 exec, %[mk]\n\t"
                       "ds_write2st64_b64 %[a], %[d0], %[d1] offset0:%[o0] offset1:%[o1]\n\t"
                       "ds_write2st64_b64 %[a], %[d2], %[d3] offset0:%[o2] offset1:%[o3]\n\t"
                       "ds_write2st64_b64 %[a], %[d4], %[d5] offset0:%[o4] offset1:%[o5]\n\t"
                       "s_mov_b64 exec, %[sv]"
                       : [sv] "=&s"(saved)
                       : [a] "v"(addr), [mk] "s"(park), [d0] "v"(pend_D[0]), [d1] "v"(pend_D[1]),
                         [d2] "v"(pend_D[2]), [d3] "v"(pend_D[3]), [d4] "v"(pend_D[4]), [d5] "v"(pend_D[5]),
                         [o0] "i"(pend_off[0]), [o1] "i"(pend_off[1]), [o2] "i"(pend_off[2]), [o3] "i"(pend_off[3]),
                         [o4] "i"(pend_off[4]), [o5] "i"(pend_off[5])
                       : "memory");
        else
          asm volatile("s_mov_b64 %[sv], exec\n\ts_mov_b64 exec, %[mk]\n\t"
                       "ds_write2st64_b64 %[a], %[d0], %[d1] offset0:%[o0] offset1:%[o1]\n\t"
                       "ds_write2st64_b64 %[a], %[d2], %[d3] offset0:%[o2] offset1:%[o3]\n\t"
                       "ds_write_b64 %[a], %[d4] offset:%[o4] * 512\n\t"
                       "s_mov_b64 exec, %[sv]"
                       : [sv] "=&s"(saved)
                       : [a] "v"(addr), [mk] "s"(park), [d0] "v"(pend_D[0]), [d1] "v"(pend_D[1]),
                         [d2] "v"(pend_D[2]), [d3] "v"(pend_D[3]), [d4] "v"(pend_D[4]),
                         [o0] "i"(pend_off[0]), [o1] "i"(pend_off[1]), [o2] "i"(pend_off[2]), [o3] "i"(pend_off[3]),
                         [o4] "i"(pend_off[4])
                       : "memory");
      }
#endif
      pend_n = 0;
    };
    auto grad_store = [&](double D, const double old, const int blk) {
#if PINN_ONETILE_SUM
      if (ONE_TILE) {
        D += dpp_mov<DPP_ROW_ROR4>(D);
        D += dpp_mov<DPP_ROW_ROR8>(D);
        pend_D[pend_n] = D; pend_off[pend_n] = blk - phase_first; ++pend_n;
        return;
      }
#else
      if (ONE_TILE) { stage_w[(blk - phase_first) * 64 + sput] = D; return; }
#endif
      D += dpp_mov<DPP_ROW_ROR8>(D);
#if PINN_GACC_ATOMIC
      if (PINN_FOLD_STAGES == 2) D += dpp_mov<DPP_ROW_ROR4>(D);
      pend_D[pend_n] = D; pend_off[pend_n] = blk * 128; ++pend_n;
      (void)old;
#else
      D += dpp_mov<DPP_ROW_ROR4>(D);
      gacc[blk * 16 + ge] = old + D;
#endif
    };
    int rel_hidden[2] = {-1, -1};
    if (ONE_TILE) {
#pragma unroll
      for (int k = 0; k < 2; ++k) {
        const int e = tid + 256 * k, bl = e >> 4, i = (e >> 2) & 3, j = e & 3;
        if (bl < 25) { const int m = bl / 5, n = bl - 5 * m; rel_hidden[k] = (4 * m + i) * FW + 4 * n + j; }
        else if (bl < 30 && i == 0) rel_hidden[k] = FW * FW + 4 * (bl - 25) + j;
      }
    }
    double* __restrict__ const row1 = part + (size_t)blockIdx.x * R;
    typedef double d2 __attribute__((ext_vector_type(2)));
    constexpr int PS_W = PINN_ONETILE_SUM ? 1 : 4;
    d2 ps_lo[2][PS_W], ps_hi[2][PS_W];
    auto phase_reads = [&](const int n_entries, const int p) {
      const double* __restrict__ const sb = gacc_all + PINN_PHASE_STAGE(p);
#pragma unroll
      for (int k = 0; k < 2; ++k) {
        if (256 * k >= n_entries) continue;
        const int e = tid + 256 * k < n_entries ? tid + 256 * k : n_entries - 1;
#if PINN_ONETILE_SUM
        ps_lo[k][0] = *reinterpret_cast<const d2*>(sb + 4 * e);
        ps_hi[k][0] = *reinterpret_cast<const d2*>(sb + 4 * e + 2);
#else
#pragma unroll
        for (int w = 0; w < 4; ++w) {
          ps_lo[k][w] = *reinterpret_cast<const d2*>(sb + w * FUSED20D_STAGE_WAVE + 4 * e);
          ps_hi[k][w] = *reinterpret_cast<const d2*>(sb + w * FUSED20D_STAGE_WAVE + 4 * e + 2);
        }
#endif
      }
    };
    auto parked_barrier = [&]() {
      if (PINN_ONETILE_SUM) asm volatile("s_waitcnt lgkmcnt(0)" ::: "memory");
      __syncthreads();
    };
    auto phase_issue = [&](const int n_entries, const int p) {
      if (PINN_ONETILE_SUM == 2) return;
      parked_barrier();
      phase_reads(n_entries, p);
    };
    auto phase_adds = [&](const int n_entries, auto to_index) {
#pragma unroll
      for (int k = 0; k < 2; ++k) {
        if (256 * k >= n_entries) continue;
        const int e = tid + 256 * k;
        const int idx = e < n_entries ? to_index(e, k) : -1;
        double v = 0.0;
#if PINN_ONETILE_SUM
        v = ((ps_lo[k][0].x + ps_lo[k][0].y) + ps_hi[k][0].x) + ps_hi[k][0].y;
#else
#pragma unroll
        for (int w = 0; w < 4; ++w) {
          const double t = (ps_lo[k][w].x + ps_lo[k][w].y) + (ps_hi[k][w].x + ps_hi[k][w].y);
          v = w == 0 ? t : v + t;
        }
#endif
#if PINN_ROW_STORE_WT
        if (idx >= 0) __hip_atomic_store(row1 + idx, v, __ATOMIC_RELAXED, __HIP_MEMORY_SCOPE_AGENT);
#else
        if (idx >= 0) row1[idx] = v;
#endif
      }
    };
    auto phase_finish = [&](const int n_entries, auto to_index) {
      if (PINN_ONETILE_SUM == 2) return;
      phase_adds(n_entries, to_index);
    };
    auto idx_dense_h = [&](const int e, int) {
      const int m = e >> 4, i = (e >> 2) & 3, j = e & 3;
      return j != 0 ? -1 : m < 5 ? nd.off_w[H] + 4 * m + i : (i == 0 ? nd.off_b[H] : -1);
    };
    const int pt = tile * 64 + wave * 16 + q;
    double sa_lam = 1.0, sa_m = 0.0, sa_v = 0.0;
    double* sa_row = nullptr;
    if constexpr (SAW && PDE == PDE_ADR) {
      const int e = pt < sd.n_all ? pt : 0;
      sa_row = sa_lam_p + PW_CONST + 3 * (e < 2 * sd.n_b ? e & ~1 : e);
      sa_lam = sa_row[0]; sa_m = sa_row[1]; sa_v = sa_row[2];
    } else
    if constexpr (SAW) {
      sa_row = sa_lam_p + SA_CONST + 3 * (pt < sd.n_all ? pt : 0);
      sa_lam = sa_row[0]; sa_m = sa_row[1]; sa_v = sa_row[2];
    }
    const double hx = __builtin_fma(sx, x - lbx, -1.0), ht = __builtin_fma(st, t - lbt, -1.0);
    {
      const int nt = tile + gridDim.x;
      if (!ONE_TILE && nt < n_tiles) { x = xs[nt * 64 + wave * 16 + q]; t = ts[nt * 64 + wave * 16 + q]; }
    }

    double in[4][5];
    double a0[5];
    agd stash[H][5][4];
    double top[5][4];
// ... 134 lines not shown
        sb[1] = fbar * adv; sb[2] = fbar; sb[3] = -kc.nu * fbar;
      } else if (cls == CLS_DATA) {
        const double dd = o[0] - tgt[pt];
        if (s == 0) lacc[64] += dd * dd * inv_nu;
        sb[0] = 2.0 * dd * inv_nu;
      } else if (cls != CLS_PAD) {
        const double du = o[0] - pu, dp = o[1] - pp;
        if (s == 0 && cls == CLS_BLO) lacc[128] += (du * du + dp * dp) * inv_nb;
        sb[0] = 2.0 * du * inv_nb; sb[1] = 2.0 * dp * inv_nb;
      } else if constexpr (pde_adr_robin(PDE)) {
        if ((unsigned)rb_j < (unsigned)rb_n) {
          typedef double d2 __attribute__((ext_vector_type(2)));
          const d2 ab = *reinterpret_cast<const d2*>(rb_ab + 2 * rb_j);
          const double r = ab.x * o[0] + ab.y * o[1] - tgt[pt];
          if (s == 0) lacc[128] += r * r * inv_nw;
          sb[0] = 2.0 * r * ab.x * inv_nw; sb[1] = 2.0 * r * ab.y * inv_nw;
        }
      }
    } else if constexpr (PDE == PDE_ADR_IDE) {
      const double pu = dpp_mov<DPP_QUAD_XOR1>(o[0]), pp = dpp_mov<DPP_QUAD_XOR1>(o[1]);
      const double* kp = adr_park;
      asm volatile("" : "+v"(kp));
      const AdrCoef<double> kc{kp[0], kp[1], kp[2], kp[3], kp[4], kp[5]};
      const double inv_nb = kp[6];
      const int cls = point_class_adr(sd, pt);
      if (cls == CLS_COL) {
        const double u = o[0], adv = kc.a0 + kc.a1 * u;
        const double f = o[2] + adv * o[1] - kc.nu * o[3] + u * (kc.r1 + u * (kc.r2 + kc.r3 * u));
        const double fbar = 2.0 * f * inv_nf;
        const double fu = fbar * u;
        const int m0 = ((s ^ 0) - 1) >> 31, m1 = ((s ^ 1) - 1) >> 31, m2 = ((s ^ 2) - 1) >> 31;
        lacc[0] += bit_pick(m0, f * f * inv_nf, bit_pick(m1, fbar * o[1], bit_pick(m2, fu * o[1], -(fbar * kc.nu) * o[3])));
        lacc[64] += bit_pick(m0, 0.0, bit_pick(m1, fu, bit_pick(m2, fu * u, fu * u * u)));
        sb[0] = fbar * (kc.a1 * o[1] + kc.r1 + u * (2.0 * kc.r2 + 3.0 * kc.r3 * u));
        sb[1] = fbar * adv; sb[2] = fbar; sb[3] = -kc.nu * fbar;
      } else if (cls == CLS_DATA) {
        const double dd = o[0] - tgt[pt];
        if (s == 0) lacc[64] += dd * dd * inv_nu;
        sb[0] = 2.0 * dd * inv_nu;
      } else if (cls != CLS_PAD) {
        const double du = o[0] - pu, dp = o[1] - pp;
        if (s == 0 && cls == CLS_BLO) lacc[128] += (du * du + dp * dp) * inv_nb;
        sb[0] = 2.0 * du * inv_nb; sb[1] = 2.0 * dp * inv_nb;
      }
    } else {
      const int cls = SAW ? (pt < sd.n_u ? CLS_DATA : pt < sd.n_all ? CLS_COL : CLS_PAD) : point_class(sd, pt);
      const bool res = (PDE == 0) ? (cls == CLS_COL) : (cls == CLS_DATA);
      double wf = inv_nf, wu = inv_nu, r2 = 0.0;
      if constexpr (SAW) {
#pragma clang fp contract(off)
        const double l2 = sa_lam * sa_lam;
        wf = inv_nf * l2; wu = inv_nu * l2;
      }
      if (res) {
        const double wgt = (PDE == 0) ? wf : inv_nu;
        const double f = o[2] + c1 * o[0] * o[1] - c2 * o[3];
        const double fbar = 2.0 * f * wgt;
        if (s == 0) {
          lacc[0] += f * f * wgt;
          if (PDE == 1) { lacc[128] += fbar * o[0] * o[1]; lacc[192] -= fbar * c2 * o[3]; }
        }
        sb[0] = fbar * c1 * o[1]; sb[1] = fbar * c1 * o[0]; sb[2] = fbar; sb[3] = -c2 * fbar;
        if constexpr (SAW) r2 = f * f;
      }
      if (cls == CLS_DATA) {
        const double dd = o[0] - tgt[pt];
        if (s == 0) lacc[64] += dd * dd * wu;
        sb[0] += 2.0 * dd * wu;
        if constexpr (SAW) r2 = dd * dd;
      }
      if constexpr (SAW) {
        if (sa_alpha != 0.0 && s == 0 && pt < sd.n_all) {
          const double* const k = sa_lam_p;
          const double g = 2.0 * sa_lam * r2 * (cls == CLS_DATA ? inv_nu : inv_nf);
          const double mi = sa_m + (1.0 - k[0]) * (g - sa_m);
          const double vi = sa_v + (1.0 - k[1]) * (g * g - sa_v);
          sa_row[0] = sa_lam + sa_alpha * mi / (sqrt(vi) + k[2]);
          sa_row[1] = mi;
          sa_row[2] = vi;
        }
      }
    }

    double ob[4][5];
    {
      double sbT[4];
#pragma unroll
      for (int c = 0; c < 4; ++c) sbT[c] = PINN_TO_POINTS(s == 0 ? sb[c] : 0.0);
      {
        double D[6] = {0.0, 0.0, 0.0, 0.0, 0.0, 0.0}, old[6];
#pragma unroll
        for (int m = 0; m < 6; ++m) old[m] = grad_fetch(BLK_H + m);
#pragma unroll
        for (int c = 0; c < 4; ++c) {
#pragma unroll
          for (int m = 0; m < 5; ++m) D[m] = mfma444(PINN_TO_POINTS(in[c][m]), sbT[c], D[m]);
        }
        D[5] = mfma444(onesA, sbT[0], 0.0);
        phase_first = BLK_H;
        stage_w = gacc_all + PINN_PHASE_STAGE(0) + wave * STAGE_WAVE_STRIDE;
#pragma unroll
        for (int m = 0; m < 6; ++m) grad_store(D[m], old[m], BLK_H + m);
        gacc_flush();
      }
#pragma unroll
      for (int n = 0; n < 5; ++n) {
        const double w = wl[nd.off_w[H] + 4 * n + s];
#pragma unroll
        for (int c = 0; c < 4; ++c) ob[c][n] = sb[c] * w;
      }
    }
    STAMP(H + 1);
#pragma unroll
    for (int d = H - 1; d >= 1; --d) {
      double zb[4][5], zbT[4][5];
      if constexpr (ONE_TILE) phase_issue(d == H - 1 ? 6 * 16 : 30 * 16, H - d - 1);
#pragma unroll
      for (int n = 0; n < 5; ++n) {
        double a, zp, zq, zr;
        if (d == H - 1) { a = top[n][0]; zp = top[n][1]; zq = top[n][2]; zr = top[n][3]; }
        else { a = agd_get(stash[d][n][0]); zp = agd_get(stash[d][n][1]); zq = agd_get(stash[d][n][2]); zr = agd_get(stash[d][n][3]); }
        preact_adjoint_d(a, zp, zq, zr, ob[0][n], ob[1][n], ob[2][n], ob[3][n], zb[0][n], zb[1][n], zb[2][n], zb[3][n]);
      }
      STAMP2(d == 4, 20);
      auto finish_prev = [&]() {
        if (d == H - 1) phase_finish(6 * 16, idx_dense_h);
        else phase_finish(30 * 16, [&](int, const int k) { return rel_hidden[k] < 0 ? -1 : nd.off_w[d + 1] + rel_hidden[k]; });
      };
      if constexpr (ONE_TILE) finish_prev();
      STAMP2(d == 4, 21);
      double cur[4] = {0.0, 0.0, 0.0, 0.0}, first_nat[4] = {0.0, 0.0, 0.0, 0.0};
      {
        double a_, zp_, zq_, zr_;
        if (d - 1 == 0) {
          a_ = a0[0]; zp_ = sx * wl[nd.off_w[0] + s]; zq_ = st * wl[nd.off_w[0] + FW + s]; zr_ = 0.0;
        } else {
          a_ = agd_get(stash[d - 1][0][0]); zp_ = agd_get(stash[d - 1][0][1]);
          zq_ = agd_get(stash[d - 1][0][2]); zr_ = agd_get(stash[d - 1][0][3]);
        }
        channels_d(a_, zp_, zq_, zr_, first_nat[0], first_nat[1], first_nat[2], first_nat[3]);
      }
      const double* __restrict__ wd = wl + nd.off_w[d] + pr;
#pragma unroll
      for (int m = 0; m < 5; ++m) {
        ob[0][m] = ob[1][m] = ob[2][m] = ob[3][m] = 0.0;
      }
      {
        auto rpat = [&](const int t) { return wd[80 * (t / 5) + 4 * (t % 5)]; };
        double Aq[4] = {rpat(0), rpat(1), 0.0, 0.0};
#pragma unroll
        for (int t = 0; t < 25; ++t) {
          const int m = t / 5, n = t - 5 * m;
          const double A = Aq[t & 3];
          if ((t & 1) == 0) {
            if (t + 2 < 25) Aq[(t + 2) & 3] = rpat(t + 2);
            if (t + 3 < 25) Aq[(t + 3) & 3] = rpat(t + 3);
          }
          if (t < 20) zbT[t / 5][t % 5] = PINN_TO_POINTS(zb[t / 5][t % 5]);
          if (t >= 20 && t < 24) cur[t - 20] = PINN_TO_POINTS(first_nat[t - 20]);
          __builtin_amdgcn_sched_barrier(0);
#pragma unroll
          for (int c = 0; c < 4; ++c) ob[c][m] = mfma444(A, zb[c][n], ob[c][m]);
          __builtin_amdgcn_sched_barrier(0);
        }
      }
      STAMP2(d == 4, 22);
      const int base = 5 + (d - 1) * 30;
      phase_first = base;
      stage_w = gacc_all + PINN_PHASE_STAGE(H - d) + wave * STAGE_WAVE_STRIDE;
#define PINN_ROTATED_INPUTS(M, O4)                                                                          \
  do {                                                                                                      \
    double a_, zp_, zq_, zr_;                                                                               \
    if (d - 1 == 0) {                                                                                       \
      const int f_ = 4 * (M) + s;                                                                           \
      a_ = a0[M]; zp_ = sx * wl[nd.off_w[0] + f_]; zq_ = st * wl[nd.off_w[0] + FW + f_]; zr_ = 0.0;         \
    } else {                                                                                                \
      a_ = agd_get(stash[d - 1][M][0]); zp_ = agd_get(stash[d - 1][M][1]);                                  \
      zq_ = agd_get(stash[d - 1][M][2]); zr_ = agd_get(stash[d - 1][M][3]);                                 \
    }                                                                                                       \
    double h_, p_, q_, r_;                                                                                  \
    channels_d(a_, zp_, zq_, zr_, h_, p_, q_, r_);                                                          \
    O4[0] = PINN_TO_POINTS(h_); O4[1] = PINN_TO_POINTS(p_);                                             \
    O4[2] = PINN_TO_POINTS(q_); O4[3] = PINN_TO_POINTS(r_);                                             \
  } while (0)
#pragma unroll
      for (int m = 0; m < 5; ++m) {
        double D[5] = {0.0, 0.0, 0.0, 0.0, 0.0}, old[5], nxt[4] = {0.0, 0.0, 0.0, 0.0};
#pragma unroll
        for (int n = 0; n < 5; ++n) old[n] = grad_fetch(base + m * 5 + n);
        if (m + 1 < 5) PINN_ROTATED_INPUTS((m + 1 < 5 ? m + 1 : 4), nxt);
#pragma unroll
        for (int c = 0; c < 4; ++c) {
#pragma unroll
          for (int n = 0; n < 5; ++n) D[n] = mfma444(cur[c], zbT[c][n], D[n]);
        }
#pragma unroll
        for (int n = 0; n < 5; ++n) grad_store(D[n], old[n], base + m * 5 + n);
        gacc_flush();
#pragma unroll
        for (int c = 0; c < 4; ++c) cur[c] = nxt[c];
        STAMP2(d == 4, 23 + m);
      }
#undef PINN_ROTATED_INPUTS
      {
        double D[5], old[5];
#pragma unroll
        for (int n = 0; n < 5; ++n) old[n] = grad_fetch(base + 25 + n);
#pragma unroll
        for (int n = 0; n < 5; ++n) D[n] = mfma444(onesA, zbT[0][n], 0.0);
#pragma unroll
        for (int n = 0; n < 5; ++n) grad_store(D[n], old[n], base + 25 + n);
        gacc_flush();
      }
      STAMP(2 * H + 1 - d);
    }
    {
      const double hxT = PINN_TO_POINTS(hx), htT = PINN_TO_POINTS(ht);
      const double Ah = i4 == 0 ? hxT : i4 == 1 ? htT : i4 == 2 ? 1.0 : 0.0;
      const double Ap = i4 == 0 ? sx : 0.0, Aq = i4 == 1 ? st : 0.0;
      double bT[3][5];
#pragma unroll
      for (int n = 0; n < 5; ++n) {
        const int f = 4 * n + s;
        double bh, bp, bq, br;
        preact_adjoint_d(a0[n], sx * wl[nd.off_w[0] + f], st * wl[nd.off_w[0] + FW + f], 0.0, ob[0][n], ob[1][n],
                         ob[2][n], ob[3][n], bh, bp, bq, br);
        bT[0][n] = PINN_TO_POINTS(bh); bT[1][n] = PINN_TO_POINTS(bp); bT[2][n] = PINN_TO_POINTS(bq);
      }
      if constexpr (ONE_TILE) {
        phase_issue(30 * 16, H - 1);
        phase_finish(30 * 16, [&](int, const int k) { return rel_hidden[k] < 0 ? -1 : nd.off_w[1] + rel_hidden[k]; });
      }
      double D[5], old[5];
#pragma unroll
      for (int n = 0; n < 5; ++n) old[n] = grad_fetch(n);
#pragma unroll
      for (int n = 0; n < 5; ++n) D[n] = mfma444(Ah, bT[0][n], 0.0);
#pragma unroll
      for (int n = 0; n < 5; ++n) D[n] = mfma444(Ap, bT[1][n], D[n]);
#pragma unroll
      for (int n = 0; n < 5; ++n) D[n] = mfma444(Aq, bT[2][n], D[n]);
      phase_first = 0;
      stage_w = gacc_all + PINN_PHASE_STAGE(H) + wave * STAGE_WAVE_STRIDE;
#pragma unroll
      for (int n = 0; n < 5; ++n) grad_store(D[n], old[n], n);
      gacc_flush();
      if constexpr (ONE_TILE) {
        auto idx_dense_0 = [&](const int e, int) {
          const int f = 4 * (e >> 4) + (e & 3), i = (e >> 2) & 3;
          return i == 0 ? nd.off_w[0] + f : i == 1 ? nd.off_w[0] + FW + f : i == 2 ? nd.off_b[0] + f : -1;
        };
        phase_issue(5 * 16, H);
        phase_finish(5 * 16, idx_dense_0);
        if constexpr (PINN_ONETILE_SUM == 2) {
          parked_barrier();
          phase_reads(6 * 16, 0);
          phase_adds(6 * 16, idx_dense_h);
#pragma unroll
          for (int d = H - 1; d >= 1; --d) {
            phase_reads(30 * 16, H - d);
            phase_adds(30 * 16, [&](int, const int k) { return rel_hidden[k] < 0 ? -1 : nd.off_w[d] + rel_hidden[k]; });
          }
          phase_reads(5 * 16, H);
          phase_adds(5 * 16, idx_dense_0);
        }
      }
    }
    if (ONE_TILE) break;
  }
  STAMP(2 * H + 1);
#undef PINN_LANE_INDICES
#undef PINN_TO_POINTS
#undef PINN_PHASE_STAGE

  {
    constexpr int NE = NBLK * 16, NIT = ONE_TILE ? 1 : (NE + 255) / 256;
    int idx[NIT];
#pragma unroll
    for (int it = 0; it < NIT; ++it) {
      const int e = tid + 256 * it;
      idx[it] = (!ONE_TILE && e < NE) ? row_index[e] : -1;
    }
    const double t0 = PDE == PDE_ADR_IDE ? row16_sum(lacc[0]) : wave_sum(lacc[0]);
    const double t1 = PDE == PDE_ADR_IDE ? row16_sum(lacc[64]) : wave_sum(lacc[64]);
    const double t2 = (PDE == 1 || pde_is_adr(PDE)) ? wave_sum(lacc[128]) : 0.0, t3 = PDE == 1 ? wave_sum(lacc[192]) : 0.0;
    double ide_mask = 0.0;
    if constexpr (PDE == PDE_ADR_IDE) ide_mask = lacc_all[wave * 256 + 192 + 7];
    __syncthreads();
    double* const scal = wl;
    if constexpr (PDE == PDE_ADR_IDE) {
      const int sl = lane >> 4;
      if ((lane & 15) == 0) {
        if (sl == 0) { scal[wave * 9 + 0] = t0; scal[wave * 9 + 1] = t1; scal[wave * 9 + 2] = t2; }
        else { scal[wave * 9 + 2 + sl] = t0; scal[wave * 9 + 5 + sl] = t1; }
      }
    } else
    if (lane == 0) { scal[wave * 4 + 0] = t0; scal[wave * 4 + 1] = t1; scal[wave * 4 + 2] = t2; scal[wave * 4 + 3] = t3; }
    __syncthreads();
    double* __restrict__ row = part + (size_t)blockIdx.x * R;
    if (!ONE_TILE) {
      double v[NIT];
#pragma unroll
      for (int it = 0; it < NIT; ++it) {
        const int e = tid + 256 * it;
        const int ee = e < NE ? e : 0;
        v[it] = ((gacc_all[ee] + gacc_all[NE + ee]) + gacc_all[2 * NE + ee]) + gacc_all[3 * NE + ee];
      }
#pragma unroll
      for (int it = 0; it < NIT; ++it)
        if (idx[it] >= 0) row[idx[it]] = v[it];
    } else if (blockIdx.x >= n_tiles) {
      for (int i = tid; i < nd.n_theta; i += 256) row[i] = 0.0;
    }
    if constexpr (PDE == PDE_ADR_IDE) {
      if (tid < 9) {
        const double v = ((scal[tid] + scal[9 + tid]) + scal[18 + tid]) + scal[27 + tid];
        if (tid < 3) row[nd.n_theta + tid] = v;
        else row[nd.n_theta - 9 + tid] = (((int)ide_mask >> (tid - 3)) & 1) ? v : 0.0;
      }
    } else
    if (tid < 4) {
      const double v = ((scal[tid] + scal[4 + tid]) + scal[8 + tid]) + scal[12 + tid];
      if (tid == 0) { row[nd.n_theta + 0] = v; if (!pde_adr_seed_block(PDE)) row[nd.n_theta + 2] = 0.0; }
      if (tid == 1) row[nd.n_theta + 1] = v;
      if (pde_adr_seed_block(PDE) && tid == 2) row[nd.n_theta + 2] = v;
      if (PDE == 1 && tid == 2) row[nd.n_net] = v;
      if (PDE == 1 && tid == 3) row[nd.n_net + 1] = v;
    }
  }
  STAMP(2 * H + 2);
}
```

pinns-tf2.0_amd/pinn_native/__init__.py:

```python
import ctypes
import os
import shutil
import subprocess

import numpy as np

_HERE = os.path.dirname(os.path.abspath(__file__))
_CSRC = os.path.join(os.path.dirname(_HERE), "csrc")
_REPO = os.path.dirname(os.path.dirname(_HERE))
LIB_PATH = os.environ.get("PINN_HIP_LIB") or os.path.join(_HERE, "libpinn_hip.so")
SOURCES = ["engine.hip", "fused20d_unit.hip", "fused20d_api.h", "fused20m_unit.hip", "fused20m_api.h", "kernels_generic.h", "kernels_fused20.h", "kernels_fused20m.h", "kernels_fused20d.h", "kernels_fused20d_kernel.h", "kernels_wide.h", "kernels_predict20.h",
           "kernels_disc.h", "kernels_sampling.h", "kernels_rad.h", "kernels_tile16.h", "kernels_tile16f.h", "kernels_xgmi.h", "kernels_optim.h", "wave.h"]
HEADER = os.path.join(_REPO, "include", "pinn_hip.h")

PDE_KINDS = {"burgers": 0, "burgers_ide": 1, "schrodinger": 2, "burgers_disc": 3, "burgers_disc_ide": 4, "adr": 5, "adr_ide": 6}


def pde_kind(name):
    if name not in PDE_KINDS:
        raise ValueError("pde must be one of %s" % sorted(PDE_KINDS))
    return PDE_KINDS[name]


DTYPES = {"f32": 0, "f64": 1, "float32": 0, "float64": 1}

ADR_COEFF_NAMES = ("a0", "a1", "nu", "r1", "r2", "r3")


def adr_trainable_mask(names_or_mask):
    if isinstance(names_or_mask, (int, np.integer)):
        return int(names_or_mask)
    if isinstance(names_or_mask, str):
        names_or_mask = [names_or_mask]
    mask = 0
    for name in names_or_mask:
        if name not in ADR_COEFF_NAMES:
            raise ValueError("unknown adr coefficient %r: choose from %s" % (name, ", ".join(ADR_COEFF_NAMES)))
        mask |= 1 << ADR_COEFF_NAMES.index(name)
    return mask


_c_double_p = ctypes.POINTER(ctypes.c_double)
_c_int_p = ctypes.POINTER(ctypes.c_int)


class PinnNativeError(RuntimeError):
    pass


COMMON_FLAGS = ["--offload-arch=gfx950", "-O3", "-std=c++17", "-fno-slp-vectorize", "-fPIC",
                "-mllvm", "-amdgpu-kernarg-preload-count=16"]
UNITS = [("engine.hip", []), ("fused20d_unit.hip", ["-mllvm", "-amdgpu-mfma-vgpr-form=1"]), ("fused20m_unit.hip", [])]


def _build_tag():
    return " ".join(COMMON_FLAGS) + " | " + " ; ".join("%s %s" % (u, " ".join(f)) for u, f in UNITS)


def _source_digest():
    import hashlib
    h = hashlib.sha256()
    for path in [os.path.join(_CSRC, s) for s in SOURCES] + [HEADER]:
        if os.path.exists(path):
            with open(path, "rb") as fh:
                h.update(fh.read())
    return h.hexdigest()


def library_digest(lib=None):
    try:
        for line in open((lib or LIB_PATH) + ".flags"):
            if line.startswith("sources-sha256 "):
                return line.split()[1]
    except OSError:
        pass
    return None


def _stale(lib=None):
    lib = lib or LIB_PATH
    if not os.path.exists(lib):
        return True
    tag = lib + ".flags"
    if os.path.exists(tag):
        lines = open(tag).read().split("\n")
        digest = [l.split(" ", 1)[1] for l in lines if l.startswith("sources-sha256 ")]
        if lines[0] != _build_tag():
            return True
        if digest:
            return digest[0] != _source_digest()
    built = os.path.getmtime(lib)
    srcs = [os.path.join(_CSRC, s) for s in SOURCES] + [HEADER]
    return any(os.path.exists(s) and os.path.getmtime(s) > built for s in srcs)

# ... 45 lines not shown
                os.replace(obj, os.path.join(_HERE, os.path.basename(obj).replace(".o", "_stamps.o" if stamps else ".o")))
        ver = subprocess.run([hipcc, "--version"], capture_output=True, text=True).stdout.strip().splitlines()
        with open(out + ".flags", "w") as fh:
            fh.write(_build_tag() + ("\n-DPINN_STAMPS" if stamps else "") + "\nsources-sha256 " + digest + "\n" +
                     "\n".join(ver[:3]) + "\n")
    return out


_LIB = None

_SIGNATURES = {
    "pinn_last_error": (ctypes.c_char_p, []),
    "pinn_abi_version": (ctypes.c_int, []),
    "pinn_device_count": (ctypes.c_int, [_c_int_p]),
    "pinn_runtime_versions": (ctypes.c_int, [_c_int_p, _c_int_p, _c_int_p]),
    "pinn_device_info": (ctypes.c_int, [ctypes.c_int, ctypes.c_char_p, ctypes.c_int, _c_int_p,
                                        ctypes.POINTER(ctypes.c_int64)]),
    "pinn_create": (ctypes.c_int, [ctypes.POINTER(ctypes.c_void_p), _c_int_p, ctypes.c_int,
                                   _c_double_p, _c_double_p, ctypes.c_int, ctypes.c_int,
                                   ctypes.c_int]),
    "pinn_destroy": (ctypes.c_int, [ctypes.c_void_p]),
    "pinn_num_params": (ctypes.c_int, [ctypes.c_void_p, ctypes.POINTER(ctypes.c_int64)]),
    "pinn_set_collocation": (ctypes.c_int, [ctypes.c_void_p, _c_double_p, ctypes.c_int64,
                                            ctypes.c_int64]),
    "pinn_set_data": (ctypes.c_int, [ctypes.c_void_p, _c_double_p, _c_double_p, ctypes.c_int64,
                                     ctypes.c_int64]),
    "pinn_set_boundary": (ctypes.c_int, [ctypes.c_void_p, _c_double_p, _c_double_p,
                                         ctypes.c_int64, ctypes.c_int64]),
    "pinn_set_pde_params": (ctypes.c_int, [ctypes.c_void_p, _c_double_p, ctypes.c_int]),
    "pinn_get_pde_params": (ctypes.c_int, [ctypes.c_void_p, _c_double_p, ctypes.c_int]),
    "pinn_set_pde_trainable": (ctypes.c_int, [ctypes.c_void_p, ctypes.c_int]),
    "pinn_set_weights": (ctypes.c_int, [ctypes.c_void_p, _c_double_p, ctypes.c_int64]),
    "pinn_get_weights": (ctypes.c_int, [ctypes.c_void_p, _c_double_p, ctypes.c_int64]),
    "pinn_loss_grad": (ctypes.c_int, [ctypes.c_void_p, _c_double_p, _c_double_p, _c_double_p]),
    "pinn_adam_init": (ctypes.c_int, [ctypes.c_void_p, ctypes.c_double, ctypes.c_double,
                                      ctypes.c_double, ctypes.c_double]),
    "pinn_adam_run_terms": (ctypes.c_int, [ctypes.c_void_p, ctypes.c_int, _c_double_p]),
    "pinn_adam_run": (ctypes.c_int, [ctypes.c_void_p, ctypes.c_int, _c_double_p]),
    "pinn_lbfgs_begin": (ctypes.c_int, [ctypes.c_void_p, ctypes.c_int, ctypes.c_double,
                                        ctypes.c_int, ctypes.c_double, ctypes.c_double,
                                        ctypes.c_double]),
    "pinn_lbfgs_run": (ctypes.c_int, [ctypes.c_void_p, ctypes.c_int, _c_int_p, _c_double_p,
                                      _c_int_p, _c_int_p]),
    "pinn_adam_enqueue": (ctypes.c_int, [ctypes.c_void_p, ctypes.c_int, _c_int_p]),
    "pinn_adam_enqueue_terms": (ctypes.c_int, [ctypes.c_void_p, ctypes.c_int, _c_int_p]),
    "pinn_adam_collect": (ctypes.c_int, [ctypes.c_void_p, ctypes.c_int, _c_double_p]),
    "pinn_lbfgs_enqueue": (ctypes.c_int, [ctypes.c_void_p, ctypes.c_int, _c_int_p]),
    "pinn_lbfgs_collect": (ctypes.c_int, [ctypes.c_void_p, ctypes.c_int, ctypes.c_int, _c_int_p, _c_double_p,
                                          _c_int_p, _c_int_p]),
    "pinn_weights_snapshot": (ctypes.c_int, [ctypes.c_void_p, ctypes.c_int]),
    "pinn_weights_restore": (ctypes.c_int, [ctypes.c_void_p, ctypes.c_int]),
    "pinn_lbfgs_get_x": (ctypes.c_int, [ctypes.c_void_p, _c_double_p, ctypes.c_int64]),
    "pinn_lbfgs_set_mode": (ctypes.c_int, [ctypes.c_void_p, ctypes.c_int]),
    "pinn_predict": (ctypes.c_int, [ctypes.c_void_p, _c_double_p, ctypes.c_int64, _c_double_p]),
    "pinn_error_l2": (ctypes.c_int, [ctypes.c_void_p, _c_double_p, _c_double_p, ctypes.c_int64, ctypes.c_int,
                                     _c_double_p]),
    "pinn_get_status": (ctypes.c_int, [ctypes.c_void_p, ctypes.POINTER(ctypes.c_int64),
                                       ctypes.POINTER(ctypes.c_int64)]),
    "pinn_residual": (ctypes.c_int, [ctypes.c_void_p, _c_double_p, ctypes.c_int64]),
    "pinn_residual_at": (ctypes.c_int, [ctypes.c_void_p, _c_double_p, ctypes.c_int64, _c_double_p]),
    "pinn_comm_xgmi_export": (ctypes.c_int, [ctypes.c_void_p, ctypes.c_int, ctypes.c_int, ctypes.c_char_p]),
    "pinn_comm_xgmi_attach": (ctypes.c_int, [ctypes.c_void_p, ctypes.c_char_p, ctypes.c_int, _c_int_p]),
    "pinn_comm_xgmi_selftest": (ctypes.c_int, [ctypes.c_void_p, _c_int_p]),
    "pinn_comm_benchmark": (ctypes.c_int, [ctypes.c_void_p, ctypes.c_int, ctypes.c_int, _c_double_p]),
    "pinn_comm_set_mode": (ctypes.c_int, [ctypes.c_void_p, ctypes.c_int]),
    "pinn_comm_get_mode": (ctypes.c_int, [ctypes.c_void_p, _c_int_p]),
    "pinn_lhs_collocation": (ctypes.c_int, [ctypes.c_void_p, ctypes.c_int64, ctypes.c_int64, ctypes.c_int64,
                                            ctypes.c_uint64]),
    "pinn_get_collocation": (ctypes.c_int, [ctypes.c_void_p, _c_double_p, ctypes.c_int64]),
    "pinn_rad_collocation": (ctypes.c_int, [ctypes.c_void_p, ctypes.c_int64, ctypes.c_int64, ctypes.c_int64,
                                            ctypes.c_int64, ctypes.c_uint64, ctypes.c_int, ctypes.c_double]),
    "pinn_disc_set_stage": (ctypes.c_int, [ctypes.c_void_p, ctypes.c_int, _c_double_p, _c_double_p,
                                           ctypes.c_int64, _c_double_p, ctypes.c_int]),
    "pinn_disc_predict": (ctypes.c_int, [ctypes.c_void_p, ctypes.c_int, _c_double_p, ctypes.c_int64,
                                         _c_double_p]),
    "pinn_comm_unique_id": (ctypes.c_int, [ctypes.c_char_p]),
    "pinn_comm_init": (ctypes.c_int, [ctypes.c_void_p, ctypes.c_char_p, ctypes.c_int,
                                      ctypes.c_int]),
    "pinn_timing_enable": (ctypes.c_int, [ctypes.c_void_p, ctypes.c_int, ctypes.c_int]),
    "pinn_timing_read": (ctypes.c_int, [ctypes.c_void_p, _c_double_p, _c_int_p]),
    "pinn_sync": (ctypes.c_int, [ctypes.c_void_p]),
    "pinn_set_kernel_path": (ctypes.c_int, [ctypes.c_void_p, ctypes.c_int]),
    "pinn_get_kernel_path": (ctypes.c_int, [ctypes.c_void_p, _c_int_p]),
    "pinn_debug_coef_stamps": (ctypes.c_int, [ctypes.POINTER(ctypes.c_longlong)]),
    "pinn_debug_t16f_stamps": (ctypes.c_int, [ctypes.POINTER(ctypes.c_longlong)]),
    "pinn_debug_t16_deal": (ctypes.c_int, [ctypes.c_int, _c_int_p]),
    "pinn_debug_stamps": (ctypes.c_int, [ctypes.c_void_p, ctypes.POINTER(ctypes.c_longlong),
                                         ctypes.c_int64, ctypes.POINTER(ctypes.c_int64)]),
    "pinn_ens_create": (ctypes.c_int, [ctypes.POINTER(ctypes.c_void_p), _c_int_p, ctypes.c_int, _c_double_p,
                                       _c_double_p, ctypes.c_int, ctypes.c_int, ctypes.c_int, ctypes.c_int]),
    "pinn_ens_destroy": (ctypes.c_int, [ctypes.c_void_p]),
    "pinn_ens_size": (ctypes.c_int, [ctypes.c_void_p, _c_int_p, ctypes.POINTER(ctypes.c_int64)]),
    "pinn_ens_set_collocation": (ctypes.c_int, [ctypes.c_void_p, _c_double_p, ctypes.c_int64, ctypes.c_int64]),
    "pinn_ens_set_data": (ctypes.c_int, [ctypes.c_void_p, _c_double_p, _c_double_p, ctypes.c_int64, ctypes.c_int64]),
    "pinn_ens_set_pde_params": (ctypes.c_int, [ctypes.c_void_p, _c_double_p, ctypes.c_int]),
    "pinn_ens_set_weights": (ctypes.c_int, [ctypes.c_void_p, _c_double_p, ctypes.c_int64]),
    "pinn_ens_get_weights": (ctypes.c_int, [ctypes.c_void_p, _c_double_p, ctypes.c_int64]),
    "pinn_ens_loss_grad": (ctypes.c_int, [ctypes.c_void_p, _c_double_p, _c_double_p, _c_double_p]),
    "pinn_ens_adam_init": (ctypes.c_int, [ctypes.c_void_p, ctypes.c_double, ctypes.c_double, ctypes.c_double,
                                          ctypes.c_double, _c_double_p]),
    "pinn_ens_adam_run": (ctypes.c_int, [ctypes.c_void_p, ctypes.c_int, _c_double_p]),
    "pinn_ens_lbfgs_begin": (ctypes.c_int, [ctypes.c_void_p, ctypes.c_int, ctypes.c_double, ctypes.c_double,
                                            ctypes.c_double, ctypes.c_double, _c_double_p, ctypes.c_int, _c_int_p]),
    "pinn_ens_lbfgs_run": (ctypes.c_int, [ctypes.c_void_p, ctypes.c_int, _c_int_p, _c_double_p, _c_int_p, _c_int_p]),
    "pinn_ens_predict": (ctypes.c_int, [ctypes.c_void_p, _c_double_p, ctypes.c_int64, _c_double_p]),
    "pinn_ens_error_l2": (ctypes.c_int, [ctypes.c_void_p, _c_double_p, _c_double_p, ctypes.c_int64, _c_double_p]),
    "pinn_ens_get_status": (ctypes.c_int, [ctypes.c_void_p, ctypes.POINTER(ctypes.c_int64),
                                           ctypes.POINTER(ctypes.c_int64)]),
    "pinn_ensk_set_collocation": (ctypes.c_int, [ctypes.c_void_p, _c_double_p, ctypes.c_int64, ctypes.c_int64]),
    "pinn_ensk_set_data": (ctypes.c_int, [ctypes.c_void_p, _c_double_p, _c_double_p, ctypes.c_int64, ctypes.c_int64]),
    "pinn_ensk_set_pde_params": (ctypes.c_int, [ctypes.c_void_p, _c_double_p, ctypes.c_int]),
    "pinn_ensk_lhs_collocation": (ctypes.c_int, [ctypes.c_void_p, ctypes.c_int64, ctypes.c_int64, ctypes.c_int64,
                                                 ctypes.POINTER(ctypes.c_uint64)]),
    "pinn_sa_set_weights": (ctypes.c_int, [ctypes.c_void_p, _c_double_p, ctypes.c_int64, _c_double_p, ctypes.c_int64]),
    "pinn_sa_get_weights": (ctypes.c_int, [ctypes.c_void_p, _c_double_p, ctypes.c_int64, _c_double_p, ctypes.c_int64]),
    "pinn_sa_adam_init": (ctypes.c_int, [ctypes.c_void_p, ctypes.c_double]),
    "pinn_sa_disable": (ctypes.c_int, [ctypes.c_void_p]),
    "pinn_pw_set": (ctypes.c_int, [ctypes.c_void_p, _c_double_p, ctypes.c_int64, _c_double_p, ctypes.c_int64,
                                   _c_double_p, ctypes.c_int64]),
    "pinn_pw_get": (ctypes.c_int, [ctypes.c_void_p, _c_double_p, ctypes.c_int64, _c_double_p, ctypes.c_int64,
                                   _c_double_p, ctypes.c_int64]),
    "pinn_pw_adam_init": (ctypes.c_int, [ctypes.c_void_p, ctypes.c_double, ctypes.c_double, ctypes.c_double]),
    "pinn_pw_disable": (ctypes.c_int, [ctypes.c_void_p]),
    "pinn_set_robin": (ctypes.c_int, [ctypes.c_void_p, _c_double_p, _c_double_p, _c_double_p, _c_double_p, ctypes.c_int64,
                                      ctypes.c_int64]),
    "pinn_robin_residual": (ctypes.c_int, [ctypes.c_void_p, _c_double_p, ctypes.c_int64]),
    "pinn_set_source": (ctypes.c_int, [ctypes.c_void_p, _c_double_p, ctypes.c_int64]),
    "pinn_set_coef_fields": (ctypes.c_int, [ctypes.c_void_p, _c_double_p, ctypes.c_int64]),
}


def exported_symbols():
    return sorted(_SIGNATURES)


def _torch_lib_dir():
    import importlib.util
    try:
        spec = importlib.util.find_spec("torch")
    except (ImportError, ValueError):
        spec = None
    if spec is None or not spec.submodule_search_locations:
        return None
    d = os.path.join(list(spec.submodule_search_locations)[0], "lib")
    return d if os.path.exists(os.path.join(d, "libamdhip64.so")) else None


def _bind_runtime():
    import sys
    policy = os.environ.get("PINN_HIP_RUNTIME", "auto").lower()
    if policy not in ("auto", "torch", "rocm"):
        raise PinnNativeError("PINN_HIP_RUNTIME must be auto, torch or rocm (got %r)" % policy)
    have_torch = "torch" in sys.modules
    if policy == "rocm":
        if have_torch:
            raise PinnNativeError("PINN_HIP_RUNTIME=rocm, but torch (with its bundled HIP runtime) is already imported "
                                  "in this process: two HIP runtimes would be mapped")
        return "rocm"
    if policy == "auto" and not have_torch and int(os.environ.get("WORLD_SIZE", "1")) <= 1:
        return "rocm"
    if have_torch:
        return "torch"
    if _torch_lib_dir() is None:
        if policy == "torch":
            raise PinnNativeError("PINN_HIP_RUNTIME=torch, but no PyTorch-ROCm wheel with a bundled runtime is installed")
        return "rocm"
# ... 417 lines not shown
        self._tickets, self._lb_uncollected = {}, 0
        self._lb_max_iter = int(max_iter)
        self._check(self._lib.pinn_lbfgs_begin(self._h, int(max_iter), lr, int(n_corr), tol_fun,
                                               tol_x, max_eval))

    def lbfgs_set_mode(self, mode):
        self._check(self._lib.pinn_lbfgs_set_mode(self._h, int(mode)))

    def lbfgs_run(self, n_iters):
        cap = max(int(n_iters), 1)
        iters = np.zeros(cap, dtype=np.int32)
        losses = np.zeros(cap, dtype=np.float64)
        n_logged, done = ctypes.c_int(0), ctypes.c_int(0)
        self._check(self._lib.pinn_lbfgs_run(self._h, int(n_iters),
                                             iters.ctypes.data_as(_c_int_p), _dp(losses),
                                             ctypes.byref(n_logged), ctypes.byref(done)))
        k = n_logged.value
        return iters[:k].copy(), losses[:k].copy(), done.value

    def lbfgs_x(self):
        x = np.empty(self.n_params, dtype=np.float64)
        self._check(self._lib.pinn_lbfgs_get_x(self._h, _dp(x), x.size))
        return x

    @staticmethod
    def comm_unique_id():
        lib = load()
        buf = ctypes.create_string_buffer(128)
        if lib.pinn_comm_unique_id(buf) != 0:
            raise PinnNativeError(lib.pinn_last_error().decode())
        return buf.raw

    def comm_init(self, unique_id, n_ranks, rank):
        self._check(self._lib.pinn_comm_init(self._h, bytes(unique_id), int(n_ranks), int(rank)))

    def comm_xgmi_export(self, n_ranks, rank):
        buf = ctypes.create_string_buffer(64)
        self._check(self._lib.pinn_comm_xgmi_export(self._h, int(n_ranks), int(rank), buf))
        return buf.raw

    def comm_xgmi_attach(self, handles):
        blob = b"".join(handles)
        ok = ctypes.c_int(0)
        self._check(self._lib.pinn_comm_xgmi_attach(self._h, blob, len(handles), ctypes.byref(ok)))
        return bool(ok.value)

    def comm_xgmi_selftest(self):
        ok = ctypes.c_int(0)
        self._check(self._lib.pinn_comm_xgmi_selftest(self._h, ctypes.byref(ok)))
        return bool(ok.value)

    def comm_benchmark(self, mode, iters=200):
        us = ctypes.c_double(0.0)
        self._check(self._lib.pinn_comm_benchmark(self._h, {"rccl": 1, "mailbox": 2}.get(mode, mode), int(iters),
                                                  ctypes.byref(us)))
        return us.value

    def comm_set_mode(self, mode):
        self._check(self._lib.pinn_comm_set_mode(self._h, {"rccl": 1, "mailbox": 2}.get(mode, mode)))

    def comm_mode(self):
        m = ctypes.c_int(0)
        self._check(self._lib.pinn_comm_get_mode(self._h, ctypes.byref(m)))
        return {0: "none", 1: "rccl", 2: "mailbox"}[m.value]

    def timing_enable(self, max_evals, every=1):
        self._check(self._lib.pinn_timing_enable(self._h, int(max_evals), int(every)))

    def timing_read(self):
        ms = np.zeros(5, dtype=np.float64)
        n = ctypes.c_int(0)
        self._check(self._lib.pinn_timing_read(self._h, _dp(ms), ctypes.byref(n)))
        return {"fwd_ms": ms[0], "sweeps_ms": ms[1], "eval_ms": ms[2], "empty_bracket_ms": ms[3],
                "kernel_exact": bool(ms[4]), "n": n.value}

    def sync(self):
        self._check(self._lib.pinn_sync(self._h))

    def set_kernel_path(self, path):
        self._check(self._lib.pinn_set_kernel_path(self._h, int(path)))

    def debug_stamps(self):
        n_wg = (2 * self.n_b + self.n_u + self.n_f + getattr(self, "n_w", 0) + 63) // 64
        buf = np.zeros((n_wg * 4, 32), dtype=np.int64)
        n = ctypes.c_int64(0)
        self._check(self._lib.pinn_debug_stamps(
            self._h, buf.ctypes.data_as(ctypes.POINTER(ctypes.c_longlong)), buf.size, ctypes.byref(n)))
        return buf[:n.value]

    def kernel_path(self):
        p = ctypes.c_int(0)
        self._check(self._lib.pinn_get_kernel_path(self._h, ctypes.byref(p)))
        return p.value


class Ensemble(object):

    MAX_MEMBERS = 64

    def __init__(self, layers, lb, ub, n_members, pde="burgers", dtype="f64", device=0):
        self._lib = load()
        self._h = ctypes.c_void_p()
        kind = pde_kind(pde)
        if dtype not in DTYPES:
            raise ValueError("dtype must be one of %s" % sorted(DTYPES))
        self.layers = [int(v) for v in layers]
        self.pde = pde
        arr = (ctypes.c_int * len(self.layers))(*self.layers)
        lb, ub = _f64(lb, (2,)), _f64(ub, (2,))
        self._check(self._lib.pinn_ens_create(ctypes.byref(self._h), arr, len(self.layers), _dp(lb), _dp(ub),
                                              kind, DTYPES[dtype], int(device), int(n_members)))
        k, n = ctypes.c_int(0), ctypes.c_int64(0)
        self._check(self._lib.pinn_ens_size(self._h, ctypes.byref(k), ctypes.byref(n)))
        self.n_members, self.n_params = k.value, n.value

    def _check(self, rc):
        if rc != 0:
            raise PinnNativeError("libpinn_hip: %s (code %d)" % (
                self._lib.pinn_last_error().decode(errors="replace"), rc))

    def close(self):
        if getattr(self, "_h", None) is not None and self._h:
            self._lib.pinn_ens_destroy(self._h)
            self._h = ctypes.c_void_p()

    def __del__(self):
        try:
            self.close()
        except Exception:
            pass

    def _per_member(self, a, what, cols):
        a = _f64(a)
        if a.ndim == 3:
            if a.shape[0] != self.n_members or a.shape[2] != cols:
                raise ValueError("%s: per-member array must be [K=%d, n, %d], got %s" % (what, self.n_members, cols,
                                                                                       a.shape))
            return a, True
        if a.size % cols:
            raise ValueError("%s: array must be [n, %d] (shared) or [K=%d, n, %d] (per member), got %s" % (
                what, cols, self.n_members, cols, a.shape))
        return a.reshape(-1, cols), False

    def set_collocation(self, X_f, n_total=None):
        X_f, per = self._per_member(X_f, "X_f", 2)
        n = X_f.shape[-2]
        nt = n if n_total is None else int(n_total)
        fn = self._lib.pinn_ensk_set_collocation if per else self._lib.pinn_ens_set_collocation
        self._check(fn(self._h, _dp(X_f), n, nt))

    def set_data(self, X_u, u, n_total=None):
        X_u, per = self._per_member(X_u, "X_u", 2)
        n = X_u.shape[-2]
        u = _f64(u)
        want = (self.n_members, n, 1) if per else (n, 1)
        if u.size != n * (self.n_members if per else 1) or (per and u.shape[:2] != want[:2]):
            raise ValueError("u: expected %s to go with X_u %s, got %s" % (want, X_u.shape, u.shape))
        u = u.reshape(want)
        nt = n if n_total is None else int(n_total)
        fn = self._lib.pinn_ensk_set_data if per else self._lib.pinn_ens_set_data
        self._check(fn(self._h, _dp(X_u), _dp(u), n, nt))

    def set_pde_params(self, *p):
        if len(p) == 1 and np.ndim(p[0]) == 1:
            nu = _f64(p[0])
            if nu.shape != (self.n_members,):
                raise ValueError("nu: per-member array must be [K=%d], got %s" % (self.n_members, nu.shape))
            self._check(self._lib.pinn_ensk_set_pde_params(self._h, _dp(nu), nu.size))
            return
        p = _f64(p)
        self._check(self._lib.pinn_ens_set_pde_params(self._h, _dp(p), p.size))

    def lhs_collocation(self, n_design, seeds, first=0, count=None):
        seeds = np.asarray(seeds)
        if seeds.shape != (self.n_members,) or not np.issubdtype(seeds.dtype, np.integer):
            raise ValueError("seeds: expected [K=%d] integers, got %s %s" % (self.n_members, seeds.shape, seeds.dtype))
        seeds = np.ascontiguousarray(seeds.astype(np.uint64))
        count = int(n_design) - int(first) if count is None else int(count)
        self._check(self._lib.pinn_ensk_lhs_collocation(self._h, int(n_design), int(first), count,
                                                        seeds.ctypes.data_as(ctypes.POINTER(ctypes.c_uint64))))

    def set_weights(self, W):
        W = _f64(W).reshape(self.n_members, self.n_params)
        self._check(self._lib.pinn_ens_set_weights(self._h, _dp(W), W.size))

    def get_weights(self):
        W = np.empty((self.n_members, self.n_params), dtype=np.float64)
        self._check(self._lib.pinn_ens_get_weights(self._h, _dp(W), W.size))
        return W

    def loss_grad(self, want_grad=True):
        losses = np.empty(self.n_members, dtype=np.float64)
        terms = np.empty((self.n_members, 3), dtype=np.float64)
        grads = np.empty((self.n_members, self.n_params), dtype=np.float64) if want_grad else None
        self._check(self._lib.pinn_ens_loss_grad(self._h, _dp(losses), _dp(grads) if want_grad else None, _dp(terms)))
        return losses, grads, terms

    def adam_init(self, lr, beta1=0.9, beta2=0.999, eps=1e-7):
        lr_k = np.broadcast_to(_f64(lr), (self.n_members,)).copy()
        self._check(self._lib.pinn_ens_adam_init(self._h, float(lr_k[0]), beta1, beta2, eps, _dp(lr_k)))

    def adam_run(self, n_steps):
        losses = np.empty((max(int(n_steps), 1), self.n_members), dtype=np.float64)
# ... 39 lines not shown
```

profiles/stamps.py:

```python
#!/usr/bin/env python3
import os
import sys

import numpy as np

ROOT = os.path.dirname(os.path.dirname(os.path.abspath(__file__)))
sys.path.insert(0, ROOT)
import bench
import burgersutil
import pinn_native


def main():
    dtype = sys.argv[1] if len(sys.argv) > 1 else "f32"
    n_f = int(sys.argv[2]) if len(sys.argv) > 2 else 10000
    np.random.seed(1234)
    r = burgersutil.prep_data(os.path.join(bench.PKG, "1d-burgers", "data", "burgers_shock.mat"), 100, n_f, noise=0.0)
    X_u, u, X_f, ub, lb = r[7], r[8], r[9], r[10], r[11]
    eng = pinn_native.Engine(bench.LAYERS, lb, ub, pde="burgers", dtype=dtype)
    eng.set_collocation(X_f)
    eng.set_data(X_u, u)
    eng.set_pde_params(bench.NU)
    eng.set_weights(bench.canonical_weights())
    for _ in range(3):
        eng.loss_grad()
    st = eng.debug_stamps().astype(np.float64)
    H = len(bench.LAYERS) - 2
    path = eng.kernel_path()
    n_st = 2 * H + 3 if path in (2, 7) else 2 * H + 2
    if len(sys.argv) > 3:
        eng.set_kernel_path(int(sys.argv[3]))
        path = eng.kernel_path()
        n_st = 2 * H + 3 if path in (2, 7) else 2 * H + 2
        st = eng.debug_stamps().astype(np.float64)
    st = st[:, :n_st].reshape(-1, 4, n_st)
    t0 = st[:, :, 0].min()
    names = (["stage weights + dense0"] + ["fwd dense %d" % d for d in range(1, H)] +
             ["output + seeds + bwd dense %d" % H] + ["bwd dense %d" % d for d in range(H - 1, 0, -1)] +
             (["bwd dense 0", "epilogue: wave sums + gradient row"] if path in (2, 7) else ["bwd dense 0 + stores"]))
    dur = np.diff(st, axis=2)
    wg_total = st[:, :, -1].max(axis=1) - st[:, :, 0].min(axis=1)
    print("# %s N_f=%d workgroups=%d  (ticks = shader cycles via s_memtime)" % (dtype, n_f, st.shape[0]))
    print("# workgroup duration ticks: min %.0f median %.0f max %.0f" % (wg_total.min(), np.median(wg_total), wg_total.max()))
    print("# first start -> last end: %.0f ticks; start spread %.0f ticks" % (
        st[:, :, -1].max() - t0, st[:, :, 0].min(axis=1).max() - t0))
    print("%-34s %10s %10s %10s" % ("phase", "median", "min", "max"))
    per = dur.max(axis=1)
    for i, nme in enumerate(names):
        print("%-34s %10.0f %10.0f %10.0f" % (nme, np.median(per[:, i]), per[:, i].min(), per[:, i].max()))
    print("%-34s %10.0f" % ("sum of medians", np.median(per, axis=0).sum()))
    if path == 7:
        full = eng.debug_stamps().astype(np.float64).reshape(-1, 4, 32)
        if np.all(full[:, :, 20:28] > 0):
            def seg(a, b):
                return np.median((full[:, :, b] - full[:, :, a]).max(axis=1))
            r0, r1 = 2 * H + 1 - 5, 2 * H + 1 - 4
            print("# reverse layer 4: adjoints + rotations %.0f | phase sum (barrier) %.0f | reverse GEMV %.0f | dW in-groups %s | bias blocks %.0f" % (
                seg(r0, 20), seg(20, 21), seg(21, 22), " ".join("%.0f" % seg(22 + m, 23 + m) for m in range(5)), seg(27, r1)))
            print("# forward layer 4: GEMV %.0f | tanh + channels + stash %.0f" % (seg(4, 29), seg(29, 5)))
    if path == 7 and st.shape[0] != (n_f + 100 + 63) // 64:
        print("# helper-wave variant (48-point tiles): mains (slowest of waves 0-2) | helper wave, medians over workgroups")
        pm, ph = dur[:, :3, :].max(axis=1), dur[:, 3, :]
        for i, nme in enumerate(names):
            print("%-34s %10.0f %10.0f" % (nme, np.median(pm[:, i]), np.median(ph[:, i])))
        full = eng.debug_stamps().astype(np.float64).reshape(-1, 4, 32)
        H_ = H
        def segm(a, b):
            return np.median((full[:, :3, b] - full[:, :3, a]).max(axis=1))
        def segh(a, b):
            return np.median(full[:, 3, b] - full[:, 3, a])
        prev = 2 * H_ + 1 - 5
        print("# layer 4, mains: adjoints+channels %.0f | wait consumed %.0f | park+flag %.0f | read back %.0f | own dW %.0f | GEMV %.0f" % (
            segm(prev, 20), segm(20, 21), segm(21, 22), segm(22, 23), segm(23, 24), segm(24, 2 * H_ + 1 - 4)))
        print("# layer 4, helper: after layer 5 .. poll %.0f | wait ready(main 0) %.0f | main 0 %.0f | main 1 %.0f | main 2 %.0f | folds+stores %.0f" % (
            segh(prev, 20), segh(20, 21), segh(21, 22), segh(22, 23), segh(23, 24), segh(24, 2 * H_ + 1 - 4)))
        print("%-34s %10.0f %10.0f" % ("whole wave (first to last stamp)", np.median((st[:, :3, -1] - st[:, :3, 0]).max(axis=1)),
                                       np.median(st[:, 3, -1] - st[:, 3, 0])))
    if path == 2:
        full = eng.debug_stamps().astype(np.float64).reshape(-1, 4, 32)
        H_ = H
        def seg(a, b):
            return np.median((full[:, :, b] - full[:, :, a]).max(axis=1))
        print("# layer 4 detail (slowest wave per workgroup, median): ")
        print("#  fwd: reads issued..gemv start %.0f | gemv %.0f | Q write + own nonlinear %.0f | barrier wait %.0f | g4 tail+barrier %.0f" % (
            seg(1 + 3, 24), seg(24, 25), seg(25, 26), seg(26, 27), seg(27, 1 + 4)))
        print("#  prologue: entry..DMA issued %.0f | ..setup done %.0f | dense 0 %.0f | barrier %.0f | layer 1 reads+gemv %.0f | "
              "nonlinear+exchange %.0f | image wait + barrier %.0f" % (
                  seg(0, 19), seg(19, 1), seg(1, 22), seg(22, 23), seg(23, 20), seg(20, 21), seg(21, 2)))
        print("#  epilogue: wave sums + first/last layer rows %.0f | dW scatter %.0f" % (seg(2 * H_ + 1, 31), seg(31, 2 * H_ + 2)))
        print("#  bwd: phase A %.0f | barrier wait %.0f | phase B (gemv + dW) %.0f | Q exchange %.0f" % (
            seg(2 * H_ + 1 - 5, 28), seg(28, 29), seg(29, 30), seg(30, 2 * H_ + 1 - 4)))
    eng.close()


if __name__ == "__main__":
    main()
```

Measured before the change: 227.3 million.

## Split f64 fused kernel into main and helper workgroups owning top-layer gradients

Adds a split launch of the fused f64 Burgers kernel. Each tile gets a main workgroup, and extra helper workgroups, one per two tiles, compute the top-layer weight gradients, so the main role skips those blocks. Parallelism grows from one workgroup per tile to about one and a half. The cost is that the helpers recompute the forward pass, and the split only applies when the grid fits within the compute-unit count. Enablement is automatic by default and controllable through PINN_F64_SPLIT.

```diff
diff --git a/include/pinn_hip.h b/include/pinn_hip.h
--- a/include/pinn_hip.h
+++ b/include/pinn_hip.h
@@ -95,6 +95,7 @@
 int pinn_sync(pinn_ctx* c);
 int pinn_set_kernel_path(pinn_ctx* c, int path);
 int pinn_get_kernel_path(pinn_ctx* c, int* path);
+int pinn_get_f64_split(pinn_ctx* c, int* split);
 int pinn_debug_stamps(pinn_ctx* c, long long* out, int64_t cap, int64_t* n_waves);
 int pinn_debug_coef_stamps(long long* out16);
 int pinn_debug_t16f_stamps(long long* out512);
diff --git a/pinns-tf2.0_amd/csrc/engine.hip b/pinns-tf2.0_amd/csrc/engine.hip
--- a/pinns-tf2.0_amd/csrc/engine.hip
+++ b/pinns-tf2.0_amd/csrc/engine.hip
@@ -132,6 +132,7 @@
   float* img = nullptr;
   int* row_index = nullptr;
   int n_cu = 256, n_wg = 0;
+  int f64_split = -1;
   void *S = nullptr, *O = nullptr, *ZA = nullptr, *ZB = nullptr, *part = nullptr;
   size_t cap_S = 0, cap_O = 0, cap_Z = 0, cap_part = 0, cap_pts = 0;
   int chunk = 0, n_rows = 0, R = 0;
@@ -769,6 +770,15 @@
                     c->stream, c->stamps, ev4 ? ev4[0] : nullptr, ev4 ? ev4[1] : nullptr};
 }
 
+static int split_plan(const pinn_ctx* c) {
+  if (!fused20d_split_built() || c->f64_split == 0) return 0;
+  if (c->path != KP_FUSED20D || c->dtype != PINN_F64 || !c->own_stream) return 0;
+  if ((c->pde != PINN_PDE_BURGERS && c->pde != PINN_PDE_BURGERS_IDE) || c->sa.on || c->pw.on) return 0;
+  const int n_tiles = c->sd.n_pad / 64;
+  const bool fits = n_tiles > 0 && c->n_wg >= n_tiles && fused20d_split_grid(n_tiles) <= c->n_cu;
+  return fits ? 1 : c->f64_split == 1 ? -1 : 0;
+}
+
 template <typename real, int PDE>
 static int launch_fused20d(pinn_ctx* c, hipEvent_t* ev4, const AdamFuse* af) {
   int rc = hipErrorInvalidValue;
@@ -777,7 +787,14 @@
     if (weighted) { if (int e = lam_prepare(c, c->sa.arr, sa_layout(c))) return e; }
     const bool pw = PDE == PDE_ADR && c->pw.on;
     if (pw) { if (int e = lam_prepare(c, c->pw.arr, pw_layout(c))) return e; }
-    const F20dLaunch a = fused20d_args(c, ev4);
+    F20dLaunch a = fused20d_args(c, ev4);
+    if constexpr (PDE == 0 || PDE == 1) {
+      const int sp = split_plan(c);
+      if (sp < 0)
+        return fail(PINN_EUNSUPPORTED, "PINN_F64_SPLIT=1: %d tiles need %d workgroups, this device has %d compute units",
+                    c->sd.n_pad / 64, fused20d_split_grid(c->sd.n_pad / 64), c->n_cu);
+      a.split = sp == 1;
+    }
     if constexpr (PDE == PDE_ADR) {
       if (pw) rc = fused20d_launch_any(a, AdrPwArgs{pde_coef<double, PDE_ADR>(c), c->pw.arr.buf, af ? af->bc_pw : 0.0});
       else rc = fused20d_launch_any(a, pde_coef<double, PDE_ADR>(c));
@@ -1469,6 +1486,11 @@
   c->R = nd.n_theta + LOSS_SLOTS;
   hipError_t e = hipStreamCreateWithFlags(&c->stream, hipStreamNonBlocking);
   if (e != hipSuccess) { delete c; return fail(PINN_EHIP, "hipStreamCreate: %s", hipGetErrorString(e)); }
+  if (const char* v = getenv("PINN_F64_SPLIT")) {
+    if (!strcmp(v, "0")) c->f64_split = 0;
+    else if (!strcmp(v, "1")) c->f64_split = 1;
+    else if (strcmp(v, "auto")) { delete c; return fail(PINN_EINVAL, "PINN_F64_SPLIT must be auto, 0 or 1 (got \"%s\")", v); }
+  }
   if (const char* v = getenv("PINN_T16_PREPASS")) {
     if (!(v[0] == '0' || v[0] == '1') || v[1]) { delete c; return fail(PINN_EINVAL, "PINN_T16_PREPASS must be 0 or 1 (got \"%s\")", v); }
     c->t16_prepass = v[0] == '1';
@@ -2689,7 +2711,8 @@
   HIPCHK(hipSetDevice(c->device));
   int rc = ensure_sets(c);
   if (rc) return rc;
-  const size_t n = (size_t)path_rows(c) * 4 * 32;
+  const int n_wgs = split_plan(c) == 1 ? fused20d_split_grid(c->sd.n_pad / 64) : path_rows(c);
+  const size_t n = (size_t)n_wgs * 4 * 32;
   REQUIRE((size_t)cap >= n, "stamp buffer too small: need %zu", n);
   if (dev_alloc(&c->stamps, n * 8)) return PINN_EHIP;
   HIPCHK(hipMemsetAsync(c->stamps, 0, n * 8, c->stream));
@@ -2745,6 +2768,18 @@
 int pinn_get_kernel_path(pinn_ctx* c, int* path) {
   REQUIRE(c && path, "null");
   *path = c->path;
+  return 0;
+}
+
+int pinn_get_f64_split(pinn_ctx* c, int* split) {
+  REQUIRE(c && split, "null");
+  HIPCHK(hipSetDevice(c->device));
+  if (int rc = ensure_sets(c)) return rc;
+  const int sp = split_plan(c);
+  if (sp < 0)
+    return fail(PINN_EUNSUPPORTED, "PINN_F64_SPLIT=1: %d tiles need %d workgroups, this device has %d compute units",
+                c->sd.n_pad / 64, fused20d_split_grid(c->sd.n_pad / 64), c->n_cu);
+  *split = sp;
   return 0;
 }
 
diff --git a/pinns-tf2.0_amd/csrc/fused20d_api.h b/pinns-tf2.0_amd/csrc/fused20d_api.h
--- a/pinns-tf2.0_amd/csrc/fused20d_api.h
+++ b/pinns-tf2.0_amd/csrc/fused20d_api.h
@@ -23,6 +23,30 @@
 
 inline bool fused20d_depth_ok(int n_hidden) { return n_hidden == 4 || n_hidden == 6 || n_hidden == 8; }
 
+enum { F20D_MAIN = 0, F20D_HELPER = 1 };
+constexpr int F20D_LOSS_SLOTS = 4;
+constexpr int F20D_WIDTH = 20;
+constexpr int f20d_layer_first(int d) { return d == 0 ? 0 : 3 * F20D_WIDTH + (d - 1) * (F20D_WIDTH + 1) * F20D_WIDTH; }
+constexpr int f20d_n_net(int H) { return f20d_layer_first(H) + F20D_WIDTH + 1; }
+constexpr int f20d_split_owner(int idx, int H, int n_tail) {
+  (void)n_tail;
+  return idx >= f20d_layer_first(H - 1) && idx < f20d_n_net(H) ? F20D_HELPER : F20D_MAIN;
+}
+constexpr bool f20d_split_ok(int H, int n_tail) {
+  const int n = f20d_n_net(H) + n_tail + F20D_LOSS_SLOTS;
+  int n_main = 0, n_helper = 0;
+  for (int i = 0; i < n; ++i) {
+    const int o = f20d_split_owner(i, H, n_tail);
+    if (o != F20D_MAIN && o != F20D_HELPER) return false;
+    const bool top = i >= f20d_layer_first(H - 1) && i < f20d_n_net(H);
+    if ((o == F20D_HELPER) != top) return false;
+    (o == F20D_HELPER ? n_helper : n_main) += 1;
+  }
+  return H >= 3 && n_main + n_helper == n && n_helper == (F20D_WIDTH + 1) * F20D_WIDTH + F20D_WIDTH + 1 && n_main > 0;
+}
+constexpr int fused20d_split_grid(int n_tiles) { return n_tiles + (n_tiles + 1) / 2; }
+constexpr bool fused20d_split_built() { return PINN_ONETILE_SUM == 0; }
+
 struct F20dLaunch {
   const NetDesc& nd;
   const SetDesc& sd;
@@ -35,6 +59,7 @@
   hipStream_t stream;
   long long* stamps;
   hipEvent_t ev_start, ev_stop;
+  bool split = false;
 };
 
 int fused20d_launch_any(int pde, const F20dLaunch& a, double nu);
diff --git a/pinns-tf2.0_amd/csrc/kernels_fused20d.h b/pinns-tf2.0_amd/csrc/kernels_fused20d.h
--- a/pinns-tf2.0_amd/csrc/kernels_fused20d.h
+++ b/pinns-tf2.0_amd/csrc/kernels_fused20d.h
@@ -101,6 +101,10 @@
 __device__ __forceinline__ double f20d_nu(const AdrPwArgs& a) { return a.k.nu; }
 __device__ __forceinline__ double f20d_nu(const AdrRobinArg<double>& a) { return a.k.nu; }
 
+static_assert(F20D_WIDTH == FW && f20d_layer_first(1) == w20_desc(8, 0).off_w[1] && f20d_layer_first(7) == w20_desc(8, 2).off_w[7] &&
+              f20d_layer_first(4) == w20_desc(4, 0).off_w[4] && f20d_n_net(6) == w20_desc(6, 2).n_net,
+              "fused20d_api.h's layer offsets are the flat layout's");
+#define PINN_F20D_SPLIT 0
 #define PINN_F20D_KERNEL k_fused20d
 #include "kernels_fused20d_kernel.h"
 #undef PINN_F20D_KERNEL
@@ -113,6 +117,14 @@
 #define PINN_F20D_KERNEL k_var20d
 #include "kernels_fused20d_kernel.h"
 #undef PINN_F20D_KERNEL
+#undef PINN_F20D_SPLIT
+#if PINN_ONETILE_SUM == 0
+#define PINN_F20D_SPLIT 1
+#define PINN_F20D_KERNEL k_split20d
+#include "kernels_fused20d_kernel.h"
+#undef PINN_F20D_KERNEL
+#undef PINN_F20D_SPLIT
+#endif
 template <int PDE, int H, bool ONE_TILE, bool ENS, bool SETS, bool SAW>
 constexpr auto f20d_kernel() {
   if constexpr (PDE == PDE_ADR_ROBIN) return &k_robin20d<PDE, H, ONE_TILE, ENS, SETS, SAW>;
@@ -135,6 +147,28 @@
     if (e != hipSuccess) return (int)e;
   }
   const int n_tiles = a.sd.n_pad / 64;
+  if (a.split) {
+    if constexpr (fused20d_split_built() && (PDE == 0 || PDE == 1) && !ENS && !SETS && !SAW) {
+#if PINN_ONETILE_SUM == 0
+      if (a.n_wg < n_tiles) return (int)hipErrorInvalidValue;
+      auto* const ks = &k_split20d<PDE, H, true, false, false, false>;
+      static unsigned long long split_attr_set = 0;
+      if (first_call_on_device(split_attr_set)) {
+        const hipError_t e = hipFuncSetAttribute((const void*)ks, hipFuncAttributeMaxDynamicSharedMemorySize, (int)lds);
+        if (e != hipSuccess) return (int)e;
+      }
+      const dim3 grid(fused20d_split_grid(n_tiles));
+      if (a.ev_start && a.ev_stop)
+        hipExtLaunchKernelGGL(ks, grid, dim3(256), lds, a.stream, a.ev_start, a.ev_stop, 0, a.th, a.xs, a.ts, a.tgt, a.part,
+                              a.row_index, a.R, n_tiles, a.lbx, a.lbt, a.sx, a.st, nu, a.sd, a.stamps, w20_desc(H, pde_n_tail(PDE)));
+      else
+        hipLaunchKernelGGL(ks, grid, dim3(256), lds, a.stream, a.th, a.xs, a.ts, a.tgt, a.part, a.row_index, a.R, n_tiles,
+                           a.lbx, a.lbt, a.sx, a.st, nu, a.sd, a.stamps, w20_desc(H, pde_n_tail(PDE)));
+      return (int)hipGetLastError();
+#endif
+    }
+    return (int)hipErrorInvalidValue;
+  }
   auto* const kern = a.n_wg >= n_tiles ? f20d_kernel<PDE, H, true, ENS, SETS, SAW>() : f20d_kernel<PDE, H, false, ENS, SETS, SAW>();
   const dim3 grid(a.n_wg, a.n_members);
   if (a.ev_start && a.ev_stop)
diff --git a/pinns-tf2.0_amd/csrc/kernels_fused20d_kernel.h b/pinns-tf2.0_amd/csrc/kernels_fused20d_kernel.h
--- a/pinns-tf2.0_amd/csrc/kernels_fused20d_kernel.h
+++ b/pinns-tf2.0_amd/csrc/kernels_fused20d_kernel.h
@@ -54,6 +54,13 @@
   double* const gacc = gacc_all + wave * (NBLK * 16);
 
   int tile = blockIdx.x;
+#if PINN_F20D_SPLIT
+  static_assert(ONE_TILE && !ENS && !SETS && !SAW && (PDE == 0 || PDE == 1) && PINN_ONETILE_SUM == 0,
+                "the split launch: one tile per workgroup, solo, Burgers kinds, unfolded phase sums");
+  static_assert(f20d_split_ok(H, pde_n_tail(PDE)), "every column of a gradient row has exactly one owner");
+  const bool helper = (int)blockIdx.x >= n_tiles;
+  if (helper) tile = 2 * ((int)blockIdx.x - n_tiles);
+#endif
   double x = 0.0, t = 0.0;
   if (tile < n_tiles) { x = xs[tile * 64 + wave * 16 + q]; t = ts[tile * 64 + wave * 16 + q]; }
 
@@ -133,7 +140,12 @@
 
   STAMP(1);
 
-  for (; tile < n_tiles; tile += gridDim.x) {
+  for (; tile < n_tiles; tile += PINN_F20D_SPLIT ? 1 : gridDim.x) {
+#if PINN_F20D_SPLIT
+    int tid_tile = threadIdx.x;
+    asm volatile("" : "+v"(tid_tile));
+    const int tid = tid_tile;
+#endif
     PINN_LANE_INDICES(tid & 63);
     auto grad_fetch = [&](const int blk) { return (ONE_TILE || PINN_GACC_ATOMIC) ? 0.0 : gacc[blk * 16 + ge]; };
     int phase_first = 0;
@@ -242,7 +254,7 @@
         else if (bl < 30 && i == 0) rel_hidden[k] = FW * FW + 4 * (bl - 25) + j;
       }
     }
-    double* __restrict__ const row1 = part + (size_t)blockIdx.x * R;
+    double* __restrict__ const row1 = part + (size_t)(PINN_F20D_SPLIT ? tile : blockIdx.x) * R;
     typedef double d2 __attribute__((ext_vector_type(2)));
     constexpr int PS_W = PINN_ONETILE_SUM ? 1 : 4;
     d2 ps_lo[2][PS_W], ps_hi[2][PS_W];
@@ -543,193 +555,28 @@
       }
     }
 
-    double ob[4][5];
-    {
-      double sbT[4];
-#pragma unroll
-      for (int c = 0; c < 4; ++c) sbT[c] = PINN_TO_POINTS(s == 0 ? sb[c] : 0.0);
-      {
-        double D[6] = {0.0, 0.0, 0.0, 0.0, 0.0, 0.0}, old[6];
-#pragma unroll
-        for (int m = 0; m < 6; ++m) old[m] = grad_fetch(BLK_H + m);
-#pragma unroll
-        for (int c = 0; c < 4; ++c) {
-#pragma unroll
-          for (int m = 0; m < 5; ++m) D[m] = mfma444(PINN_TO_POINTS(in[c][m]), sbT[c], D[m]);
-        }
-        D[5] = mfma444(onesA, sbT[0], 0.0);
-        phase_first = BLK_H;
-        stage_w = gacc_all + PINN_PHASE_STAGE(0) + wave * STAGE_WAVE_STRIDE;
-#pragma unroll
-        for (int m = 0; m < 6; ++m) grad_store(D[m], old[m], BLK_H + m);
-        gacc_flush();
-      }
-#pragma unroll
-      for (int n = 0; n < 5; ++n) {
-        const double w = wl[nd.off_w[H] + 4 * n + s];
-#pragma unroll
-        for (int c = 0; c < 4; ++c) ob[c][n] = sb[c] * w;
-      }
-    }
-    STAMP(H + 1);
-#pragma unroll
-    for (int d = H - 1; d >= 1; --d) {
-      double zb[4][5], zbT[4][5];
-      if constexpr (ONE_TILE) phase_issue(d == H - 1 ? 6 * 16 : 30 * 16, H - d - 1);
-#pragma unroll
-      for (int n = 0; n < 5; ++n) {
-        double a, zp, zq, zr;
-        if (d == H - 1) { a = top[n][0]; zp = top[n][1]; zq = top[n][2]; zr = top[n][3]; }
-        else { a = agd_get(stash[d][n][0]); zp = agd_get(stash[d][n][1]); zq = agd_get(stash[d][n][2]); zr = agd_get(stash[d][n][3]); }
-        preact_adjoint_d(a, zp, zq, zr, ob[0][n], ob[1][n], ob[2][n], ob[3][n], zb[0][n], zb[1][n], zb[2][n], zb[3][n]);
-      }
-      STAMP2(d == 4, 20);
-      auto finish_prev = [&]() {
-        if (d == H - 1) phase_finish(6 * 16, idx_dense_h);
-        else phase_finish(30 * 16, [&](int, const int k) { return rel_hidden[k] < 0 ? -1 : nd.off_w[d + 1] + rel_hidden[k]; });
-      };
-      if constexpr (ONE_TILE) finish_prev();
-      STAMP2(d == 4, 21);
-      double cur[4] = {0.0, 0.0, 0.0, 0.0}, first_nat[4] = {0.0, 0.0, 0.0, 0.0};
-      {
-        double a_, zp_, zq_, zr_;
-        if (d - 1 == 0) {
-          a_ = a0[0]; zp_ = sx * wl[nd.off_w[0] + s]; zq_ = st * wl[nd.off_w[0] + FW + s]; zr_ = 0.0;
-        } else {
-          a_ = agd_get(stash[d - 1][0][0]); zp_ = agd_get(stash[d - 1][0][1]);
-          zq_ = agd_get(stash[d - 1][0][2]); zr_ = agd_get(stash[d - 1][0][3]);
-        }
-        channels_d(a_, zp_, zq_, zr_, first_nat[0], first_nat[1], first_nat[2], first_nat[3]);
-      }
-      const double* __restrict__ wd = wl + nd.off_w[d] + pr;
-#pragma unroll
-      for (int m = 0; m < 5; ++m) {
-        ob[0][m] = ob[1][m] = ob[2][m] = ob[3][m] = 0.0;
-      }
-      {
-        auto rpat = [&](const int t) { return wd[80 * (t / 5) + 4 * (t % 5)]; };
-        double Aq[4] = {rpat(0), rpat(1), 0.0, 0.0};
-#pragma unroll
-        for (int t = 0; t < 25; ++t) {
-          const int m = t / 5, n = t - 5 * m;
-          const double A = Aq[t & 3];
-          if ((t & 1) == 0) {
-            if (t + 2 < 25) Aq[(t + 2) & 3] = rpat(t + 2);
-            if (t + 3 < 25) Aq[(t + 3) & 3] = rpat(t + 3);
-          }
-          if (t < 20) zbT[t / 5][t % 5] = PINN_TO_POINTS(zb[t / 5][t % 5]);
-          if (t >= 20 && t < 24) cur[t - 20] = PINN_TO_POINTS(first_nat[t - 20]);
-          __builtin_amdgcn_sched_barrier(0);
-#pragma unroll
-          for (int c = 0; c < 4; ++c) ob[c][m] = mfma444(A, zb[c][n], ob[c][m]);
-          __builtin_amdgcn_sched_barrier(0);
-        }
-      }
-      STAMP2(d == 4, 22);
-      const int base = 5 + (d - 1) * 30;
-      phase_first = base;
-      stage_w = gacc_all + PINN_PHASE_STAGE(H - d) + wave * STAGE_WAVE_STRIDE;
-#define PINN_ROTATED_INPUTS(M, O4)                                                                          \
-  do {                                                                                                      \
-    double a_, zp_, zq_, zr_;                                                                               \
-    if (d - 1 == 0) {                                                                                       \
-      const int f_ = 4 * (M) + s;                                                                           \
-      a_ = a0[M]; zp_ = sx * wl[nd.off_w[0] + f_]; zq_ = st * wl[nd.off_w[0] + FW + f_]; zr_ = 0.0;         \
-    } else {                                                                                                \
-      a_ = agd_get(stash[d - 1][M][0]); zp_ = agd_get(stash[d - 1][M][1]);                                  \
-      zq_ = agd_get(stash[d - 1][M][2]); zr_ = agd_get(stash[d - 1][M][3]);                                 \
-    }                                                                                                       \
-    double h_, p_, q_, r_;                                                                                  \
-    channels_d(a_, zp_, zq_, zr_, h_, p_, q_, r_);                                                          \
-    O4[0] = PINN_TO_POINTS(h_); O4[1] = PINN_TO_POINTS(p_);                                             \
-    O4[2] = PINN_TO_POINTS(q_); O4[3] = PINN_TO_POINTS(r_);                                             \
-  } while (0)
-#pragma unroll
-      for (int m = 0; m < 5; ++m) {
-        double D[5] = {0.0, 0.0, 0.0, 0.0, 0.0}, old[5], nxt[4] = {0.0, 0.0, 0.0, 0.0};
-#pragma unroll
-        for (int n = 0; n < 5; ++n) old[n] = grad_fetch(base + m * 5 + n);
-        if (m + 1 < 5) PINN_ROTATED_INPUTS((m + 1 < 5 ? m + 1 : 4), nxt);
-#pragma unroll
-        for (int c = 0; c < 4; ++c) {
-#pragma unroll
-          for (int n = 0; n < 5; ++n) D[n] = mfma444(cur[c], zbT[c][n], D[n]);
-        }
-#pragma unroll
-        for (int n = 0; n < 5; ++n) grad_store(D[n], old[n], base + m * 5 + n);
-        gacc_flush();
-#pragma unroll
-        for (int c = 0; c < 4; ++c) cur[c] = nxt[c];
-        STAMP2(d == 4, 23 + m);
-      }
-#undef PINN_ROTATED_INPUTS
-      {
-        double D[5], old[5];
-#pragma unroll
-        for (int n = 0; n < 5; ++n) old[n] = grad_fetch(base + 25 + n);
-#pragma unroll
-        for (int n = 0; n < 5; ++n) D[n] = mfma444(onesA, zbT[0][n], 0.0);
-#pragma unroll
-        for (int n = 0; n < 5; ++n) grad_store(D[n], old[n], base + 25 + n);
-        gacc_flush();
-      }
-      STAMP(2 * H + 1 - d);
-    }
-    {
-      const double hxT = PINN_TO_POINTS(hx), htT = PINN_TO_POINTS(ht);
-      const double Ah = i4 == 0 ? hxT : i4 == 1 ? htT : i4 == 2 ? 1.0 : 0.0;
-      const double Ap = i4 == 0 ? sx : 0.0, Aq = i4 == 1 ? st : 0.0;
-      double bT[3][5];
-#pragma unroll
-      for (int n = 0; n < 5; ++n) {
-        const int f = 4 * n + s;
-        double bh, bp, bq, br;
-        preact_adjoint_d(a0[n], sx * wl[nd.off_w[0] + f], st * wl[nd.off_w[0] + FW + f], 0.0, ob[0][n], ob[1][n],
-                         ob[2][n], ob[3][n], bh, bp, bq, br);
-        bT[0][n] = PINN_TO_POINTS(bh); bT[1][n] = PINN_TO_POINTS(bp); bT[2][n] = PINN_TO_POINTS(bq);
-      }
-      if constexpr (ONE_TILE) {
-        phase_issue(30 * 16, H - 1);
-        phase_finish(30 * 16, [&](int, const int k) { return rel_hidden[k] < 0 ? -1 : nd.off_w[1] + rel_hidden[k]; });
-      }
-      double D[5], old[5];
-#pragma unroll
-      for (int n = 0; n < 5; ++n) old[n] = grad_fetch(n);
-#pragma unroll
-      for (int n = 0; n < 5; ++n) D[n] = mfma444(Ah, bT[0][n], 0.0);
-#pragma unroll
-      for (int n = 0; n < 5; ++n) D[n] = mfma444(Ap, bT[1][n], D[n]);
-#pragma unroll
-      for (int n = 0; n < 5; ++n) D[n] = mfma444(Aq, bT[2][n], D[n]);
-      phase_first = 0;
-      stage_w = gacc_all + PINN_PHASE_STAGE(H) + wave * STAGE_WAVE_STRIDE;
-#pragma unroll
-      for (int n = 0; n < 5; ++n) grad_store(D[n], old[n], n);
-      gacc_flush();
-      if constexpr (ONE_TILE) {
-        auto idx_dense_0 = [&](const int e, int) {
-          const int f = 4 * (e >> 4) + (e & 3), i = (e >> 2) & 3;
-          return i == 0 ? nd.off_w[0] + f : i == 1 ? nd.off_w[0] + FW + f : i == 2 ? nd.off_b[0] + f : -1;
-        };
-        phase_issue(5 * 16, H);
-        phase_finish(5 * 16, idx_dense_0);
-        if constexpr (PINN_ONETILE_SUM == 2) {
-          parked_barrier();
-          phase_reads(6 * 16, 0);
-          phase_adds(6 * 16, idx_dense_h);
-#pragma unroll
-          for (int d = H - 1; d >= 1; --d) {
-            phase_reads(30 * 16, H - d);
-            phase_adds(30 * 16, [&](int, const int k) { return rel_hidden[k] < 0 ? -1 : nd.off_w[d] + rel_hidden[k]; });
-          }
-          phase_reads(5 * 16, H);
-          phase_adds(5 * 16, idx_dense_0);
-        }
-      }
-    }
+#if PINN_F20D_SPLIT
+    if (helper) {
+#define PINN_F20D_ROLE 2
+#include "kernels_fused20d_reverse.h"
+#undef PINN_F20D_ROLE
+    } else {
+#define PINN_F20D_ROLE 1
+#include "kernels_fused20d_reverse.h"
+#undef PINN_F20D_ROLE
+    }
+    if (helper && !(tile & 1)) continue;
+#else
+#define PINN_F20D_ROLE 0
+#include "kernels_fused20d_reverse.h"
+#undef PINN_F20D_ROLE
+#endif
     if (ONE_TILE) break;
   }
   STAMP(2 * H + 1);
+#if PINN_F20D_SPLIT
+  if (helper) return;
+#endif
 #undef PINN_LANE_INDICES
 #undef PINN_TO_POINTS
 #undef PINN_PHASE_STAGE
diff --git a/pinns-tf2.0_amd/csrc/kernels_fused20d_reverse.h b/pinns-tf2.0_amd/csrc/kernels_fused20d_reverse.h
--- /dev/null
+++ b/pinns-tf2.0_amd/csrc/kernels_fused20d_reverse.h
@@ -0,0 +1,204 @@
+#define PINN_ROLE_OWNS(COL)                                                                                           \
+  (PINN_F20D_ROLE == 0 || f20d_split_owner((COL), H, pde_n_tail(PDE)) == (PINN_F20D_ROLE == 2 ? F20D_HELPER : F20D_MAIN))
+    double ob[4][5];
+    if (PINN_F20D_ROLE == 2) {
+      const int nt = tile + 1;
+      if (!(tile & 1) && nt < n_tiles) { x = xs[nt * 64 + wave * 16 + q]; t = ts[nt * 64 + wave * 16 + q]; }
+    }
+    {
+      if (PINN_ROLE_OWNS(nd_const.off_w[H])) {
+      double sbT[4];
+#pragma unroll
+      for (int c = 0; c < 4; ++c) sbT[c] = PINN_TO_POINTS(s == 0 ? sb[c] : 0.0);
+      {
+        double D[6] = {0.0, 0.0, 0.0, 0.0, 0.0, 0.0}, old[6];
+#pragma unroll
+        for (int m = 0; m < 6; ++m) old[m] = grad_fetch(BLK_H + m);
+#pragma unroll
+        for (int c = 0; c < 4; ++c) {
+#pragma unroll
+          for (int m = 0; m < 5; ++m) D[m] = mfma444(PINN_TO_POINTS(in[c][m]), sbT[c], D[m]);
+        }
+        D[5] = mfma444(onesA, sbT[0], 0.0);
+        phase_first = BLK_H;
+        stage_w = gacc_all + PINN_PHASE_STAGE(0) + wave * STAGE_WAVE_STRIDE;
+#pragma unroll
+        for (int m = 0; m < 6; ++m) grad_store(D[m], old[m], BLK_H + m);
+        gacc_flush();
+      }
+      }
+#pragma unroll
+      for (int n = 0; n < 5; ++n) {
+        const double w = wl[nd.off_w[H] + 4 * n + s];
+#pragma unroll
+        for (int c = 0; c < 4; ++c) ob[c][n] = sb[c] * w;
+      }
+    }
+    STAMP(H + 1);
+#pragma unroll
+    for (int d = H - 1; d >= (PINN_F20D_ROLE == 2 ? H - 1 : 1); --d) {
+      const bool prev_here = PINN_ROLE_OWNS(nd_const.off_w[d + 1]), dw_here = PINN_ROLE_OWNS(nd_const.off_w[d]);
+      double zb[4][5], zbT[4][5];
+      if constexpr (ONE_TILE) { if (prev_here) phase_issue(d == H - 1 ? 6 * 16 : 30 * 16, H - d - 1); }
+#pragma unroll
+      for (int n = 0; n < 5; ++n) {
+        double a, zp, zq, zr;
+        if (d == H - 1) { a = top[n][0]; zp = top[n][1]; zq = top[n][2]; zr = top[n][3]; }
+        else { a = agd_get(stash[d][n][0]); zp = agd_get(stash[d][n][1]); zq = agd_get(stash[d][n][2]); zr = agd_get(stash[d][n][3]); }
+        preact_adjoint_d(a, zp, zq, zr, ob[0][n], ob[1][n], ob[2][n], ob[3][n], zb[0][n], zb[1][n], zb[2][n], zb[3][n]);
+      }
+      STAMP2(d == 4, 20);
+      auto finish_prev = [&]() {
+        if (d == H - 1) phase_finish(6 * 16, idx_dense_h);
+        else phase_finish(30 * 16, [&](int, const int k) { return rel_hidden[k] < 0 ? -1 : nd.off_w[d + 1] + rel_hidden[k]; });
+      };
+      if constexpr (ONE_TILE) { if (prev_here) finish_prev(); }
+      STAMP2(d == 4, 21);
+      double cur[4] = {0.0, 0.0, 0.0, 0.0}, first_nat[4] = {0.0, 0.0, 0.0, 0.0};
+      if (dw_here) {
+        double a_, zp_, zq_, zr_;
+        if (d - 1 == 0) {
+          a_ = a0[0]; zp_ = sx * wl[nd.off_w[0] + s]; zq_ = st * wl[nd.off_w[0] + FW + s]; zr_ = 0.0;
+        } else {
+          a_ = agd_get(stash[d - 1][0][0]); zp_ = agd_get(stash[d - 1][0][1]);
+          zq_ = agd_get(stash[d - 1][0][2]); zr_ = agd_get(stash[d - 1][0][3]);
+        }
+        channels_d(a_, zp_, zq_, zr_, first_nat[0], first_nat[1], first_nat[2], first_nat[3]);
+      }
+      const double* __restrict__ wd = wl + nd.off_w[d] + pr;
+#pragma unroll
+      for (int m = 0; m < 5; ++m) {
+        ob[0][m] = ob[1][m] = ob[2][m] = ob[3][m] = 0.0;
+      }
+      {
+        auto rpat = [&](const int t) { return wd[80 * (t / 5) + 4 * (t % 5)]; };
+        double Aq[4] = {rpat(0), rpat(1), 0.0, 0.0};
+#pragma unroll
+        for (int t = 0; t < 25; ++t) {
+          const int m = t / 5, n = t - 5 * m;
+          const double A = Aq[t & 3];
+          if ((t & 1) == 0) {
+            if (t + 2 < 25) Aq[(t + 2) & 3] = rpat(t + 2);
+            if (t + 3 < 25) Aq[(t + 3) & 3] = rpat(t + 3);
+          }
+          if (t < 20 && dw_here) zbT[t / 5][t % 5] = PINN_TO_POINTS(zb[t / 5][t % 5]);
+          if (t >= 20 && t < 24 && dw_here) cur[t - 20] = PINN_TO_POINTS(first_nat[t - 20]);
+          __builtin_amdgcn_sched_barrier(0);
+          if (PINN_F20D_ROLE != 2) {
+#pragma unroll
+          for (int c = 0; c < 4; ++c) ob[c][m] = mfma444(A, zb[c][n], ob[c][m]);
+          }
+          __builtin_amdgcn_sched_barrier(0);
+        }
+      }
+      STAMP2(d == 4, 22);
+      if (dw_here) {
+      const int base = 5 + (d - 1) * 30;
+      phase_first = base;
+      stage_w = gacc_all + PINN_PHASE_STAGE(H - d) + wave * STAGE_WAVE_STRIDE;
+#define PINN_ROTATED_INPUTS(M, O4)                                                                          \
+  do {                                                                                                      \
+    double a_, zp_, zq_, zr_;                                                                               \
+    if (d - 1 == 0) {                                                                                       \
+      const int f_ = 4 * (M) + s;                                                                           \
+      a_ = a0[M]; zp_ = sx * wl[nd.off_w[0] + f_]; zq_ = st * wl[nd.off_w[0] + FW + f_]; zr_ = 0.0;         \
+    } else {                                                                                                \
+      a_ = agd_get(stash[d - 1][M][0]); zp_ = agd_get(stash[d - 1][M][1]);                                  \
+      zq_ = agd_get(stash[d - 1][M][2]); zr_ = agd_get(stash[d - 1][M][3]);                                 \
+    }                                                                                                       \
+    double h_, p_, q_, r_;                                                                                  \
+    channels_d(a_, zp_, zq_, zr_, h_, p_, q_, r_);                                                          \
+    O4[0] = PINN_TO_POINTS(h_); O4[1] = PINN_TO_POINTS(p_);                                             \
+    O4[2] = PINN_TO_POINTS(q_); O4[3] = PINN_TO_POINTS(r_);                                             \
+  } while (0)
+#pragma unroll
+      for (int m = 0; m < 5; ++m) {
+        double D[5] = {0.0, 0.0, 0.0, 0.0, 0.0}, old[5], nxt[4] = {0.0, 0.0, 0.0, 0.0};
+#pragma unroll
+        for (int n = 0; n < 5; ++n) old[n] = grad_fetch(base + m * 5 + n);
+        if (m + 1 < 5) PINN_ROTATED_INPUTS((m + 1 < 5 ? m + 1 : 4), nxt);
+#pragma unroll
+        for (int c = 0; c < 4; ++c) {
+#pragma unroll
+          for (int n = 0; n < 5; ++n) D[n] = mfma444(cur[c], zbT[c][n], D[n]);
+        }
+#pragma unroll
+        for (int n = 0; n < 5; ++n) grad_store(D[n], old[n], base + m * 5 + n);
+        gacc_flush();
+#pragma unroll
+        for (int c = 0; c < 4; ++c) cur[c] = nxt[c];
+        STAMP2(d == 4, 23 + m);
+      }
+#undef PINN_ROTATED_INPUTS
+      {
+        double D[5], old[5];
+#pragma unroll
+        for (int n = 0; n < 5; ++n) old[n] = grad_fetch(base + 25 + n);
+#pragma unroll
+        for (int n = 0; n < 5; ++n) D[n] = mfma444(onesA, zbT[0][n], 0.0);
+#pragma unroll
+        for (int n = 0; n < 5; ++n) grad_store(D[n], old[n], base + 25 + n);
+        gacc_flush();
+      }
+      }
+      STAMP(2 * H + 1 - d);
+    }
+    if (PINN_F20D_ROLE == 2) {
+      phase_issue(30 * 16, 1);
+      phase_finish(30 * 16, [&](int, const int k) { return rel_hidden[k] < 0 ? -1 : nd.off_w[H - 1] + rel_hidden[k]; });
+      STAMP((tile & 1) ? 31 : 19);
+    }
+    if (PINN_F20D_ROLE != 2) {
+      const double hxT = PINN_TO_POINTS(hx), htT = PINN_TO_POINTS(ht);
+      const double Ah = i4 == 0 ? hxT : i4 == 1 ? htT : i4 == 2 ? 1.0 : 0.0;
+      const double Ap = i4 == 0 ? sx : 0.0, Aq = i4 == 1 ? st : 0.0;
+      double bT[3][5];
+#pragma unroll
+      for (int n = 0; n < 5; ++n) {
+        const int f = 4 * n + s;
+        double bh, bp, bq, br;
+        preact_adjoint_d(a0[n], sx * wl[nd.off_w[0] + f], st * wl[nd.off_w[0] + FW + f], 0.0, ob[0][n], ob[1][n],
+                         ob[2][n], ob[3][n], bh, bp, bq, br);
+        bT[0][n] = PINN_TO_POINTS(bh); bT[1][n] = PINN_TO_POINTS(bp); bT[2][n] = PINN_TO_POINTS(bq);
+      }
+      if constexpr (ONE_TILE) {
+        static_assert(PINN_F20D_ROLE == 2 || (PINN_ROLE_OWNS(nd_const.off_w[1]) && PINN_ROLE_OWNS(nd_const.off_w[0])), "the bottom of the sweep is the main role's");
+        phase_issue(30 * 16, H - 1);
+        phase_finish(30 * 16, [&](int, const int k) { return rel_hidden[k] < 0 ? -1 : nd.off_w[1] + rel_hidden[k]; });
+      }
+      double D[5], old[5];
+#pragma unroll
+      for (int n = 0; n < 5; ++n) old[n] = grad_fetch(n);
+#pragma unroll
+      for (int n = 0; n < 5; ++n) D[n] = mfma444(Ah, bT[0][n], 0.0);
+#pragma unroll
+      for (int n = 0; n < 5; ++n) D[n] = mfma444(Ap, bT[1][n], D[n]);
+#pragma unroll
+      for (int n = 0; n < 5; ++n) D[n] = mfma444(Aq, bT[2][n], D[n]);
+      phase_first = 0;
+      stage_w = gacc_all + PINN_PHASE_STAGE(H) + wave * STAGE_WAVE_STRIDE;
+#pragma unroll
+      for (int n = 0; n < 5; ++n) grad_store(D[n], old[n], n);
+      gacc_flush();
+      if constexpr (ONE_TILE) {
+        auto idx_dense_0 = [&](const int e, int) {
+          const int f = 4 * (e >> 4) + (e & 3), i = (e >> 2) & 3;
+          return i == 0 ? nd.off_w[0] + f : i == 1 ? nd.off_w[0] + FW + f : i == 2 ? nd.off_b[0] + f : -1;
+        };
+        phase_issue(5 * 16, H);
+        phase_finish(5 * 16, idx_dense_0);
+        if constexpr (PINN_ONETILE_SUM == 2) {
+          parked_barrier();
+          phase_reads(6 * 16, 0);
+          phase_adds(6 * 16, idx_dense_h);
+#pragma unroll
+          for (int d = H - 1; d >= 1; --d) {
+            phase_reads(30 * 16, H - d);
+            phase_adds(30 * 16, [&](int, const int k) { return rel_hidden[k] < 0 ? -1 : nd.off_w[d] + rel_hidden[k]; });
+          }
+          phase_reads(5 * 16, H);
+          phase_adds(5 * 16, idx_dense_0);
+        }
+      }
+    }
+#undef PINN_ROLE_OWNS
diff --git a/pinns-tf2.0_amd/pinn_native/__init__.py b/pinns-tf2.0_amd/pinn_native/__init__.py
--- a/pinns-tf2.0_amd/pinn_native/__init__.py
+++ b/pinns-tf2.0_amd/pinn_native/__init__.py
@@ -9,7 +9,7 @@
 _CSRC = os.path.join(os.path.dirname(_HERE), "csrc")
 _REPO = os.path.dirname(os.path.dirname(_HERE))
 LIB_PATH = os.environ.get("PINN_HIP_LIB") or os.path.join(_HERE, "libpinn_hip.so")
-SOURCES = ["engine.hip", "fused20d_unit.hip", "fused20d_api.h", "fused20m_unit.hip", "fused20m_api.h", "kernels_generic.h", "kernels_fused20.h", "kernels_fused20m.h", "kernels_fused20d.h", "kernels_fused20d_kernel.h", "kernels_wide.h", "kernels_predict20.h",
+SOURCES = ["engine.hip", "fused20d_unit.hip", "fused20d_api.h", "fused20m_unit.hip", "fused20m_api.h", "kernels_generic.h", "kernels_fused20.h", "kernels_fused20m.h", "kernels_fused20d.h", "kernels_fused20d_kernel.h", "kernels_fused20d_reverse.h", "kernels_wide.h", "kernels_predict20.h",
            "kernels_disc.h", "kernels_sampling.h", "kernels_rad.h", "kernels_tile16.h", "kernels_tile16f.h", "kernels_xgmi.h", "kernels_optim.h", "wave.h"]
 HEADER = os.path.join(_REPO, "include", "pinn_hip.h")
 
@@ -221,6 +221,7 @@
     "pinn_sync": (ctypes.c_int, [ctypes.c_void_p]),
     "pinn_set_kernel_path": (ctypes.c_int, [ctypes.c_void_p, ctypes.c_int]),
     "pinn_get_kernel_path": (ctypes.c_int, [ctypes.c_void_p, _c_int_p]),
+    "pinn_get_f64_split": (ctypes.c_int, [ctypes.c_void_p, _c_int_p]),
     "pinn_debug_coef_stamps": (ctypes.c_int, [ctypes.POINTER(ctypes.c_longlong)]),
     "pinn_debug_t16f_stamps": (ctypes.c_int, [ctypes.POINTER(ctypes.c_longlong)]),
     "pinn_debug_t16_deal": (ctypes.c_int, [ctypes.c_int, _c_int_p]),
@@ -804,6 +805,7 @@
 
     def debug_stamps(self):
         n_wg = (2 * self.n_b + self.n_u + self.n_f + getattr(self, "n_w", 0) + 63) // 64
+        n_wg += (n_wg + 1) // 2
         buf = np.zeros((n_wg * 4, 32), dtype=np.int64)
         n = ctypes.c_int64(0)
         self._check(self._lib.pinn_debug_stamps(
@@ -814,6 +816,12 @@
         p = ctypes.c_int(0)
         self._check(self._lib.pinn_get_kernel_path(self._h, ctypes.byref(p)))
         return p.value
+
+    @property
+    def f64_split(self):
+        p = ctypes.c_int(0)
+        self._check(self._lib.pinn_get_f64_split(self._h, ctypes.byref(p)))
+        return bool(p.value)
 
 
 class Ensemble(object):
@@ -841,6 +849,8 @@
             raise PinnNativeError("libpinn_hip: %s (code %d)" % (
                 self._lib.pinn_last_error().decode(errors="replace"), rc))
 
+    f64_split = False
+
     def close(self):
         if getattr(self, "_h", None) is not None and self._h:
             self._lib.pinn_ens_destroy(self._h)
diff --git a/profiles/stamps.py b/profiles/stamps.py
--- a/profiles/stamps.py
+++ b/profiles/stamps.py
@@ -33,6 +33,10 @@
         path = eng.kernel_path()
         n_st = 2 * H + 3 if path in (2, 7) else 2 * H + 2
         st = eng.debug_stamps().astype(np.float64)
+    helpers = None
+    if path == 7 and eng.f64_split:
+        n_main = (eng.n_u + eng.n_f + 63) // 64
+        helpers, st = st[4 * n_main:].reshape(-1, 4, 32), st[:4 * n_main]
     st = st[:, :n_st].reshape(-1, 4, n_st)
     t0 = st[:, :, 0].min()
     names = (["stage weights + dense0"] + ["fwd dense %d" % d for d in range(1, H)] +
@@ -49,8 +53,30 @@
     for i, nme in enumerate(names):
         print("%-34s %10.0f %10.0f %10.0f" % (nme, np.median(per[:, i]), per[:, i].min(), per[:, i].max()))
     print("%-34s %10.0f" % ("sum of medians", np.median(per, axis=0).sum()))
+    if helpers is not None:
+        print("# split launch: the table above is the MAIN role (no dense-%d blocks, reverse layer %d without its gradient blocks);"
+              " %d helper workgroups:" % (H, H - 1, helpers.shape[0]))
+        two = helpers[:, 0, 31] > 0
+        h_total = helpers[:, :, 2 * H + 1].max(axis=1) - helpers[:, :, 0].min(axis=1)
+        print("# helper duration ticks: min %.0f median %.0f max %.0f; %d of them served two tiles" % (
+            h_total.min(), np.median(h_total), h_total.max(), int(two.sum())))
+        hh = helpers[two] if two.any() else helpers
+        end_last = hh[:, :, 31] if two.any() else hh[:, :, 19]
+        start_last = hh[:, :, 19] if two.any() else hh[:, :, 1]
+        def hseg(a, b):
+            return np.median((b - a).max(axis=1))
+        rows = [("stage weights", hseg(hh[:, :, 0], hh[:, :, 1]))]
+        if two.any():
+            rows.append(("first tile (whole)", hseg(hh[:, :, 1], hh[:, :, 19])))
+        rows.append(("last tile: dense 0 + fwd dense 1", hseg(start_last, hh[:, :, 2])))
+        rows += [("last tile: fwd dense %d" % d, hseg(hh[:, :, d], hh[:, :, 1 + d])) for d in range(2, H)]
+        rows.append(("last tile: output + seeds + dW %d" % H, hseg(hh[:, :, H], hh[:, :, H + 1])))
+        rows.append(("last tile: layer %d adjoints + dW" % (H - 1), hseg(hh[:, :, H + 1], hh[:, :, H + 2])))
+        rows.append(("last tile: last phase sum", hseg(hh[:, :, H + 2], end_last)))
+        for nme, v in rows:
+            print("%-34s %10.0f" % (nme, v))
     if path == 7:
-        full = eng.debug_stamps().astype(np.float64).reshape(-1, 4, 32)
+        full = eng.debug_stamps().astype(np.float64).reshape(-1, 4, 32)[:st.shape[0]]
         if np.all(full[:, :, 20:28] > 0):
             def seg(a, b):
                 return np.median((full[:, :, b] - full[:, :, a]).max(axis=1))
```

Result: faster. 237.4 million, median of 6 (+4.5%).
